# bghira/universal-metal-flash-attention

Measured on AMD Instinct MI355X. Metric: SDPA fwd TFLOPS (bf16) + int8 speedup, B=1 H=24 S=4096 D=128, 1/2/4/8 GPU, higher is better.
Workload: dtype bf16

## Files before the change

universal-metal-flash-attention_amd/csrc/fa_aux.hip:

```cpp
#include "fa_common.h"
#include "kernels.h"

namespace umfa {

template <typename T>
__global__ __launch_bounds__(256) void rope_rotate_kernel(RopeParams p) {
    const uint32_t chunks_per_row = p.D / 8;
    const uint64_t total = (uint64_t)p.B * p.H * p.S * chunks_per_row;
    for (uint64_t i = (uint64_t)blockIdx.x * 256 + threadIdx.x; i < total; i += (uint64_t)gridDim.x * 256) {
        const uint32_t ch = (uint32_t)(i % chunks_per_row);
        const uint64_t row = i / chunks_per_row;
        const uint32_t s = (uint32_t)(row % p.S);
        const uint64_t bh = row / p.S;
        const uint32_t h = (uint32_t)(bh % p.H), b = (uint32_t)(bh / p.H);
        const T* src = (const T*)p.src + (int64_t)b * p.src_batch_stride + (int64_t)h * p.src_head_stride +
                       (int64_t)s * p.src_seq_stride + ch * 8;
        T* dst = (T*)p.dst + row * p.D + ch * 8;
        const int64_t t = (int64_t)b * p.table_batch_stride + (int64_t)s * p.D + ch * 8;
        float x[8];
        if constexpr (sizeof(T) == 2) {
            typedef T T8 __attribute__((ext_vector_type(8)));
            const T8 v = *(const T8*)src;
#pragma unroll
            for (int j = 0; j < 8; ++j) x[j] = (float)v[j];
        } else {
            const f32x4 a = *(const f32x4*)src, c = *(const f32x4*)(src + 4);
#pragma unroll
            for (int j = 0; j < 4; ++j) { x[j] = a[j]; x[4 + j] = c[j]; }
        }
        const f32x4 c0 = *(const f32x4*)(p.cos_table + t), c1 = *(const f32x4*)(p.cos_table + t + 4);
        const f32x4 s0 = *(const f32x4*)(p.sin_table + t), s1 = *(const f32x4*)(p.sin_table + t + 4);
        float y[8];
        rope_rotate8(x, c0, c1, s0, s1, p.negate_sin != 0, y);
        if constexpr (sizeof(T) == 2) {
            typedef T T8 __attribute__((ext_vector_type(8)));
            T8 o;
#pragma unroll
            for (int j = 0; j < 8; ++j) o[j] = (T)y[j];
            *(T8*)dst = o;
        } else {
            *(f32x4*)dst = f32x4{y[0], y[1], y[2], y[3]};
            *(f32x4*)(dst + 4) = f32x4{y[4], y[5], y[6], y[7]};
        }
    }
}

template <typename T>
__global__ __launch_bounds__(256) void rope_rotate_pair_kernel(RopeParams p) {
    const uint32_t pairs = p.D / 2;
    const uint64_t total = (uint64_t)p.B * p.H * p.S * pairs;
    for (uint64_t i = (uint64_t)blockIdx.x * 256 + threadIdx.x; i < total; i += (uint64_t)gridDim.x * 256) {
        const uint32_t pr = (uint32_t)(i % pairs);
        const uint64_t row = i / pairs;
        const uint32_t s = (uint32_t)(row % p.S);
        const uint64_t bh = row / p.S;
        const uint32_t h = (uint32_t)(bh % p.H), b = (uint32_t)(bh / p.H);
        const T* src = (const T*)p.src + (int64_t)b * p.src_batch_stride + (int64_t)h * p.src_head_stride +
                       (int64_t)s * p.src_seq_stride + pr * 2;
        T* dst = (T*)p.dst + row * p.D + pr * 2;
        const int64_t t = (int64_t)b * p.table_batch_stride + (int64_t)s * p.D + pr * 2;
        const float c = p.cos_table[t];
        float sn = p.sin_table[t];
        if (p.negate_sin) sn = -sn;
        const float x0 = (float)src[0], x1 = (float)src[1];
        dst[0] = (T)(x0 * c - x1 * sn);
        dst[1] = (T)(x1 * c + x0 * sn);
    }
}

template <typename T>
static hipError_t launch_rope_t(const RopeParams& p, hipStream_t stream) {
    const bool vec = p.D % 8 == 0 && p.src_batch_stride % 8 == 0 && p.src_head_stride % 8 == 0 &&
                     p.src_seq_stride % 8 == 0 && p.table_batch_stride % 4 == 0 && ((uintptr_t)p.src & 15) == 0 &&
                     ((uintptr_t)p.dst & 15) == 0 && ((uintptr_t)p.cos_table & 15) == 0 && ((uintptr_t)p.sin_table & 15) == 0;
    const uint64_t work = (uint64_t)p.B * p.H * p.S * (vec ? p.D / 8 : p.D / 2);
    if (work == 0) return hipSuccess;
    const unsigned grid = (unsigned)((work + 255) / 256 < 2048 * 8 ? (work + 255) / 256 : 2048 * 8);
    if (vec) hipLaunchKernelGGL(rope_rotate_kernel<T>, dim3(grid), dim3(256), 0, stream, p);
    else hipLaunchKernelGGL(rope_rotate_pair_kernel<T>, dim3(grid), dim3(256), 0, stream, p);
    return hipGetLastError();
}

// ... 322 lines not shown
    if (wid >= total) return;
    const uint32_t tile = (uint32_t)(wid % T);
    const uint32_t rb = (uint32_t)((wid / T) % nrb64);
    const uint32_t slab = (uint32_t)(wid / ((uint64_t)T * nrb64));
    const uint32_t hm = slab % Hm, bm = slab / Hm;
    const uint8_t* base = (const uint8_t*)p.mask + (int64_t)bm * p.ms[0] + (int64_t)hm * p.ms[1];
    bool all_open = (uint64_t)tile * 64 + 64 <= p.Skv, any_open = false;
    uint32_t w[2];
    if constexpr (VEC16) {
        uint8_t* st = stage[wv];
        typedef unsigned u32x4 __attribute__((ext_vector_type(4)));
#pragma unroll
        for (int ps = 0; ps < 4; ++ps) {
            const uint32_t r = 16 * ps + (lane >> 2), c = lane & 3, row = rb * 64 + r, key0 = tile * 64 + 16 * c;
            u32x4 v = {0u, 0u, 0u, 0u};
            if (row < p.Sq && key0 < p.Skv) v = *(const u32x4*)(base + (int64_t)row * p.ms[2] + key0);
            *(u32x4*)(st + r * 80 + 16 * c) = v;
        }
        __builtin_amdgcn_fence(__ATOMIC_RELEASE, "wavefront");
        __builtin_amdgcn_wave_barrier();
        __builtin_amdgcn_fence(__ATOMIC_ACQUIRE, "wavefront");
#pragma unroll
        for (int qb = 0; qb < 2; ++qb) {
            const uint32_t r = 32 * qb + ql;
            uint32_t word = 0;
#pragma unroll
            for (int kb = 0; kb < 2; ++kb)
#pragma unroll
                for (int g = 0; g < 4; ++g) {
                    const uint32_t four = *(const uint32_t*)(st + r * 80 + 32 * kb + 8 * g + 4 * hi);
#pragma unroll
                    for (int e = 0; e < 4; ++e) word |= ((four >> (8 * e)) & 0xffu) ? 1u << (16 * kb + 4 * g + e) : 0u;
                }
            if (p.causal) word &= causal_word(rb * 64 + r, tile, hi);
            if (rb * 64 + r < p.Sq) {
                all_open = all_open && word == 0xffffffffu;
                any_open = any_open || word != 0;
            }
            w[qb] = word;
        }
    } else {
        const bool vec4 = p.ms[3] == 1 && ((p.ms[0] | p.ms[1] | p.ms[2]) & 3) == 0 && ((uintptr_t)p.mask & 3) == 0;
#pragma unroll
        for (int qb = 0; qb < 2; ++qb) {
            const uint32_t row = rb * 64 + 32 * qb + ql;
            uint32_t word = 0;
            if (row < p.Sq) {
                const uint8_t* rp = base + (int64_t)row * p.ms[2];
#pragma unroll
                for (int kb = 0; kb < 2; ++kb)
#pragma unroll
                    for (int g = 0; g < 4; ++g) {
                        const uint32_t key0 = tile * 64 + 32 * kb + 8 * g + 4 * hi;
                        uint32_t four = 0;
                        if (vec4 && key0 + 4 <= p.Skv) {
                            four = *(const uint32_t*)(rp + key0);
                        } else {
#pragma unroll
                            for (int e = 0; e < 4; ++e)
                                if (key0 + e < p.Skv) four |= (uint32_t)rp[(int64_t)(key0 + e) * p.ms[3]] << (8 * e);
                        }
#pragma unroll
                        for (int e = 0; e < 4; ++e) word |= ((four >> (8 * e)) & 0xffu) ? 1u << (16 * kb + 4 * g + e) : 0u;
                    }
                if (p.causal) word &= causal_word(row, tile, hi);
                all_open = all_open && word == 0xffffffffu;
                any_open = any_open || word != 0;
            }
            w[qb] = word;
        }
    }
    uint32_t* dst = bits + ((wid * 2) * 64 + lane);
    dst[0] = w[0];
    dst[64] = w[1];
    const bool open = __builtin_amdgcn_ballot_w64(any_open) != 0, full = __builtin_amdgcn_ballot_w64(!all_open) == 0;
    if (lane == 0) wflag[wid] = !open ? 1 : (full ? 2 : 0);
}

template <bool VEC16>
__global__ __launch_bounds__(256) void mask_pack_kernel(MaskPackArgs p) {
    mask_pack_body<VEC16>(p, blockIdx.x);
}

constexpr uint32_t VH_WORDS = 128, VH_DEPART = 64, VH_SCALE = 65, VH_AMAX = 66;
__device__ __forceinline__ int vscale_exponent(unsigned amax_bits) {
    if (amax_bits == 0) return 0;
    int E = (int)(amax_bits >> 7);
    E = E > 254 ? 254 : E;
    const int e = (E ? E - 127 : -126) - 15;
    return e < -100 ? -100 : e;
}
__device__ __forceinline__ unsigned bf16x8_amax(const unsigned (&r)[4], unsigned amax) {
#pragma unroll
    for (int j = 0; j < 4; ++j) {
        const unsigned a = r[j] & 0x7fff7fffu, m2 = (a & 0xffffu) > (a >> 16) ? (a & 0xffffu) : (a >> 16);
        amax = amax > m2 ? amax : m2;
    }
    return amax;
}
__device__ __forceinline__ unsigned wave_umax(unsigned x) {
#pragma unroll
    for (int off = 32; off > 0; off >>= 1) {
        const unsigned o2 = (unsigned)__shfl_xor((int)x, off, 64);
        x = x > o2 ? x : o2;
    }
    return x;
}
__device__ __forceinline__ unsigned block_amax(unsigned amax, unsigned* wmax) {
    amax = wave_umax(amax);
    if ((threadIdx.x & 63) == 0) wmax[threadIdx.x >> 6] = amax;
    __syncthreads();
    unsigned m = wmax[0];
    for (int w = 1; w < 4; ++w) m = m > wmax[w] ? m : wmax[w];
    return m;
}

struct CastRowsArgs {
    const uint16_t* src;
    int64_t sb, sh, ss;
    _Float16* dst;
    uint32_t H, S, D8, chunks;
    uint32_t* hdr;
    uint32_t wait_ticks;
};
template <int U, bool FUSED>
__device__ __forceinline__ void cast_rows_body(const CastRowsArgs& a, const uint32_t block) {
    const uint16_t* __restrict__ src = a.src;
    _Float16* __restrict__ dst = a.dst;
    uint32_t* __restrict__ hdr = a.hdr;
    const int64_t sb = a.sb, sh = a.sh, ss = a.ss;
    const uint32_t H = a.H, S = a.S, D8 = a.D8, chunks = a.chunks;
    typedef unsigned u32x4 __attribute__((ext_vector_type(4)));
    __shared__ unsigned wmax[4], slab_amax;
    const uint32_t bh = block / chunks, chunk = block - bh * chunks, b = bh / H, h = bh - b * H;
    const uint32_t rpw = 256u / D8;
    const uint32_t tr = threadIdx.x / D8, c = threadIdx.x - tr * D8;
    const uint32_t row0 = chunk * (U * rpw) + tr;
    const uint16_t* sp = src + (int64_t)b * sb + (int64_t)h * sh + 8 * c;
    _Float16* dp = dst + ((int64_t)bh * S) * (8 * D8) + 8 * c;
    uint32_t* const hw = hdr + VH_WORDS * (size_t)bh;
    u32x4 raw[U];
#pragma unroll
    for (int u = 0; u < U; ++u) {
        const uint32_t r = row0 + u * rpw;
        raw[u] = r < S && tr < rpw ? __builtin_nontemporal_load((const u32x4*)(sp + (int64_t)r * ss)) : u32x4{0, 0, 0, 0};
    }
    unsigned amax;
    if constexpr (FUSED) {
        amax = 0;
#pragma unroll
        for (int u = 0; u < U; ++u) {
            const unsigned r4[4] = {raw[u][0], raw[u][1], raw[u][2], raw[u][3]};
            amax = bf16x8_amax(r4, amax);
        }
        amax = block_amax(amax, wmax);
        if (threadIdx.x < 64) {
            if (threadIdx.x == 0) __hip_atomic_store(hw + chunk, 0x80000000u | amax, __ATOMIC_RELAXED, __HIP_MEMORY_SCOPE_AGENT);
            const uint64_t t_in = __builtin_amdgcn_s_memrealtime();
            unsigned f;
            bool served = true;
            for (;;) {
                f = threadIdx.x < chunks ? __hip_atomic_load(hw + threadIdx.x, __ATOMIC_RELAXED, __HIP_MEMORY_SCOPE_AGENT) : 0x80000000u;
                if (__builtin_amdgcn_ballot_w64((f & 0x80000000u) == 0) == 0) break;
                if (__builtin_amdgcn_s_memrealtime() - t_in >= a.wait_ticks) { served = false; break; }
                __builtin_amdgcn_s_sleep(2);
            }
            f = wave_umax(f & 0x7fffffffu);
            if (threadIdx.x == 0) slab_amax = served ? f : 0xffffffffu;
        }
        __syncthreads();
        if (slab_amax == 0xffffffffu) {
            for (uint32_t r = tr; r < S && tr < rpw; r += rpw) {
                const u32x4 v = *(const u32x4*)(sp + (int64_t)r * ss);
                const unsigned r4[4] = {v[0], v[1], v[2], v[3]};
                amax = bf16x8_amax(r4, amax);
            }
            __syncthreads();
            amax = block_amax(amax, wmax);
        } else {
            amax = slab_amax;
        }
    } else {
        amax = hw[VH_AMAX];
    }
    const int e = vscale_exponent(amax);
    const float mul = __uint_as_float((unsigned)(127 - e) << 23);
#pragma unroll
    for (int u = 0; u < U; ++u) {
        const uint32_t r = row0 + u * rpw;
        u32x4 o;
#pragma unroll
        for (int j = 0; j < 4; ++j) {
            const float lo = __uint_as_float(raw[u][j] << 16) * mul, hi = __uint_as_float(raw[u][j] & 0xffff0000u) * mul;
            asm("v_cvt_pk_f16_f32 %0, %1, %2" : "=v"(o[j]) : "v"(lo), "v"(hi));
        }
        if (r < S && tr < rpw) *(u32x4*)(dp + (int64_t)r * (8 * D8)) = o;
    }
    if (threadIdx.x < 64) {
        unsigned d = 0;
        if (threadIdx.x == 0) d = __hip_atomic_fetch_add(hw + VH_DEPART, 1u, __ATOMIC_RELAXED, __HIP_MEMORY_SCOPE_AGENT);
        d = (unsigned)__builtin_amdgcn_readfirstlane((int)d);
        if (d == chunks - 1) {
            if (FUSED && threadIdx.x < chunks) __hip_atomic_store(hw + threadIdx.x, 0u, __ATOMIC_RELAXED, __HIP_MEMORY_SCOPE_AGENT);
            if (threadIdx.x == 0) {
                hw[VH_SCALE] = (unsigned)(127 + e) << 23;
                __hip_atomic_store(hw + VH_DEPART, 0u, __ATOMIC_RELAXED, __HIP_MEMORY_SCOPE_AGENT);
                if (!FUSED) __hip_atomic_store(hw + VH_AMAX, 0u, __ATOMIC_RELAXED, __HIP_MEMORY_SCOPE_AGENT);
            }
        }
    }
}

template <int U, bool FUSED>
__global__ __launch_bounds__(256) void cast_rows_bf16_f16_kernel(CastRowsArgs a) {
    cast_rows_body<U, FUSED>(a, blockIdx.x);
}

template <int U, bool VEC16>
__global__ __launch_bounds__(256) void cast_rows_and_mask_pack_kernel(CastRowsArgs a, uint32_t cast_blocks, MaskPackArgs mk) {
    if (blockIdx.x < cast_blocks) cast_rows_body<U, true>(a, blockIdx.x);
    else mask_pack_body<VEC16>(mk, blockIdx.x - cast_blocks);
}

template <int U>
__global__ __launch_bounds__(256) void vamax_rows_kernel(const uint16_t* __restrict__ src, int64_t sb, int64_t sh, int64_t ss, uint32_t H, uint32_t S,
                                                         uint32_t D8, uint32_t chunks, uint32_t* __restrict__ hdr) {
    typedef unsigned u32x4 __attribute__((ext_vector_type(4)));
    __shared__ unsigned wmax[4];
    const uint32_t bh = blockIdx.x / chunks, chunk = blockIdx.x - bh * chunks, b = bh / H, h = bh - b * H;
    const uint32_t rpw = 256u / D8, tr = threadIdx.x / D8, c = threadIdx.x - tr * D8;
    const uint32_t row0 = chunk * (U * rpw) + tr;
    const uint16_t* sp = src + (int64_t)b * sb + (int64_t)h * sh + 8 * c;
    unsigned amax = 0;
#pragma unroll
    for (int u = 0; u < U; ++u) {
        const uint32_t r = row0 + u * rpw;
        const u32x4 v = r < S && tr < rpw ? *(const u32x4*)(sp + (int64_t)r * ss) : u32x4{0, 0, 0, 0};
        const unsigned r4[4] = {v[0], v[1], v[2], v[3]};
        amax = bf16x8_amax(r4, amax);
    }
    amax = block_amax(amax, wmax);
    if (threadIdx.x == 0 && amax) (void)__hip_atomic_fetch_max(hdr + VH_WORDS * (size_t)bh + VH_AMAX, amax, __ATOMIC_RELAXED, __HIP_MEMORY_SCOPE_AGENT);
}

template <int U>
static hipError_t launch_cast_rows_u(const void* src, const int64_t* strides, void* dst, uint32_t B, uint32_t H, uint32_t S, uint32_t D, uint32_t* hdr,
                                     hipStream_t stream, MaskPackArgs* mk) {
    const uint32_t D8 = D / 8, rpw = 256u / D8;
    const uint64_t chunks = ((uint64_t)S + U * rpw - 1) / (U * rpw), grid = (uint64_t)B * H * chunks;
    if (grid > 0x7fffffffull) return hipErrorInvalidValue;
    const bool fused = chunks <= 64 && !tuning().cast_two_pass.load(std::memory_order_relaxed);
    const CastRowsArgs a = {(const uint16_t*)src, strides[0], strides[1], strides[2], (_Float16*)dst, H, S, D8, (uint32_t)chunks, hdr,
                            (uint32_t)std::min<int64_t>(std::max(tuning().cast_wait_us.load(std::memory_order_relaxed), 0), 1000000) * 100u};
    if (fused) {
        if (mk && mk->total) {
            const unsigned g2 = (unsigned)((mk->total + 3) / 4);
            if (grid + g2 > 0x7fffffffull) return hipErrorInvalidValue;
            if (mk->vec16) hipLaunchKernelGGL((cast_rows_and_mask_pack_kernel<U, true>), dim3((unsigned)grid + g2), dim3(256), 0, stream, a, (unsigned)grid, *mk);
            else hipLaunchKernelGGL((cast_rows_and_mask_pack_kernel<U, false>), dim3((unsigned)grid + g2), dim3(256), 0, stream, a, (unsigned)grid, *mk);
            mk->done = true;
        } else {
            hipLaunchKernelGGL((cast_rows_bf16_f16_kernel<U, true>), dim3((unsigned)grid), dim3(256), 0, stream, a);
        }
    } else {
        hipLaunchKernelGGL(vamax_rows_kernel<U>, dim3((unsigned)grid), dim3(256), 0, stream, (const uint16_t*)src, strides[0], strides[1], strides[2], H, S,
                           D8, (uint32_t)chunks, hdr);
        hipLaunchKernelGGL((cast_rows_bf16_f16_kernel<U, false>), dim3((unsigned)grid), dim3(256), 0, stream, a);
    }
    return hipGetLastError();
}

static hipError_t launch_cast_rows_any(const void* src, const int64_t* strides, void* dst, uint32_t B, uint32_t H, uint32_t S, uint32_t D,
                                       uint32_t* hdr, hipStream_t stream, MaskPackArgs* mk) {
    if (!src || !dst || !hdr || (D & 7) || D > 2048 || strides[3] != 1 || (strides[0] | strides[1] | strides[2]) % 8 || ((uintptr_t)src & 15)) return hipErrorInvalidValue;
    if ((int64_t)B * H * S * D == 0) return hipSuccess;
    const uint32_t rpw = 256u / (D / 8);
    const uint64_t wg16 = (uint64_t)B * H * (((uint64_t)S + 16 * rpw - 1) / (16 * rpw));
    const int lab = tuning().cast_u.load(std::memory_order_relaxed);
    const uint64_t chunks16 = ((uint64_t)S + 16 * rpw - 1) / (16 * rpw);
    if (lab == 32 || (!lab && chunks16 > 64 && chunks16 <= 128)) return launch_cast_rows_u<32>(src, strides, dst, B, H, S, D, hdr, stream, mk);
    if (lab == 4 || (!lab && wg16 < (uint64_t)device_cu_count())) return launch_cast_rows_u<4>(src, strides, dst, B, H, S, D, hdr, stream, mk);
    return launch_cast_rows_u<16>(src, strides, dst, B, H, S, D, hdr, stream, mk);
}

hipError_t launch_bwd16_rowc(const float* lse, const float* dvec, float* rowc, int64_t n, const float* d_mul, hipStream_t stream) {
    if (n == 0) return hipSuccess;
    const unsigned grid = (unsigned)((n + 255) / 256 < 4096 ? (n + 255) / 256 : 4096);
    hipLaunchKernelGGL(bwd16_rowc_kernel, dim3(grid), dim3(256), 0, stream, lse, dvec, rowc, n, d_mul);
    return hipGetLastError();
}

hipError_t launch_dequant(const DequantParams& p, hipStream_t stream) {
    if (!p.src || (!p.dst && !p.dst16) || p.H_src == 0 || p.H_dst % p.H_src) return hipErrorInvalidValue;
    const int64_t n = (int64_t)p.B * p.H_dst * p.S * p.D;
// ... 612 lines not shown
```

universal-metal-flash-attention_amd/csrc/fa_common.h:

```cpp
#pragma once
#include <hip/hip_runtime.h>
#include <stdint.h>

namespace umfa {

typedef float f32x16 __attribute__((ext_vector_type(16)));
typedef float f32x4 __attribute__((ext_vector_type(4)));
typedef short s16x8 __attribute__((ext_vector_type(8)));
typedef short s16x4 __attribute__((ext_vector_type(4)));
typedef _Float16 f16x8 __attribute__((ext_vector_type(8)));
typedef __bf16 bf16x8 __attribute__((ext_vector_type(8)));
typedef int i32x4 __attribute__((ext_vector_type(4)));
typedef int i32x16 __attribute__((ext_vector_type(16)));

enum Prec : int { P_FP16 = 0, P_BF16 = 1, P_FP32 = 2, P_INT8 = 3, P_INT4 = 4 };
enum MaskKind : int { MK_NONE = 0, MK_BOOL = 1, MK_F32 = 2, MK_F16 = 3, MK_BF16 = 4,
                      MK_WINDOW = 5  };

#define UMFA_LOG2E 1.4426950408889634f
#define UMFA_LN2 0.6931471805599453f

struct FwdParams {
    const void* q;
    const void* k;
    const void* v;
    void* o;
    float* lse;
    const void* mask;
    int64_t qs[4], ks[4], vs[4];
    int64_t os[2];
    int64_t ms[4];
    uint32_t B, H, Sq, Skv, D;
    float scale;
    int causal;
    int mask_kind;
    int in_prec;
    int out_prec;
    uint32_t n_full;
    uint32_t nsplit;
    float* part_buf;
    uint32_t* part_cnt;
    const uint8_t* mask_flags;
    uint32_t mf_bs, mf_hs;
    uint32_t mf_nrb, mf_ntiles;
    uint32_t win_left, win_right;
    const uint32_t* mk_bits;
    const uint32_t* mk_list;
    const uint32_t* mk_cnt;
    uint32_t mk_bs, mk_hs, mk_nrb64, mk_T;
    const uint32_t* mk_prefix;
    const float* rope_cos;
    const float* rope_sin;
    int64_t rope_tb;
    int pv16;
    const float* vsc;
    uint32_t vsc_bs, vsc_hs;
    uint32_t decode_form;
    uint32_t cbal;
    uint32_t cbal_delta;
    const uint32_t* guard;
    uint32_t guard_want;
    uint32_t mask_padded;
};

__device__ __forceinline__ void rope_rotate8(const float (&x)[8], const f32x4& c0, const f32x4& c1, const f32x4& s0,
                                             const f32x4& s1, bool negate_sin, float (&y)[8]) {
    const float cs[4] = {c0[0], c0[2], c1[0], c1[2]};
    float sn[4] = {s0[0], s0[2], s1[0], s1[2]};
#pragma unroll
    for (int k = 0; k < 4; ++k) {
        if (negate_sin) sn[k] = -sn[k];
        y[2 * k] = __builtin_fmaf(x[2 * k], cs[k], -__fmul_rn(x[2 * k + 1], sn[k]));
        y[2 * k + 1] = __builtin_fmaf(x[2 * k + 1], cs[k], __fmul_rn(x[2 * k], sn[k]));
    }
#pragma unroll
    for (int j = 0; j < 8; ++j) asm volatile("" : "+v"(y[j]));
}

template <typename T, typename V8>
__device__ __forceinline__ V8 rope_fragment(V8 v, const float* __restrict__ cos_t, const float* __restrict__ sin_t, int64_t at) {
    float x[8], y[8];
#pragma unroll
    for (int j = 0; j < 8; ++j) x[j] = (float)v[j];
    const f32x4 c0 = *(const f32x4*)(cos_t + at), c1 = *(const f32x4*)(cos_t + at + 4);
    const f32x4 s0 = *(const f32x4*)(sin_t + at), s1 = *(const f32x4*)(sin_t + at + 4);
    rope_rotate8(x, c0, c1, s0, s1, false, y);
    V8 o;
#pragma unroll
    for (int j = 0; j < 8; ++j) o[j] = (T)y[j];
    return o;
}

struct BwdParams {
    const void* dout;
    const void* q;
    const void* k;
    const void* v;
    const float* o;
    const float* lse;
    float* dq;
    float* dk;
    float* dv;
    float* dvec;
    float* rowc;
    const void* mask;
    uint32_t B, H, Sq, Skv, D;
    float scale;
    int causal;
    int in_prec;
    int dout_prec;
    int grad_in_type;
    int o_in_type;
    int phases;
    uint32_t Hkv;
    int dkdv_fp32;
    void* ds;
    int ds_lab;
    const float* units;
    int64_t ms[4];
    int mask_kind;
    uint32_t win_left, win_right;
    const uint8_t* mask_flags;
    uint32_t mf_bs, mf_hs, mf_nrb, mf_ntiles;
};

inline void bwd_dense_f32_mask(BwdParams& p, const void* mask) {
    p.mask = mask;
    p.mask_kind = mask ? MK_F32 : MK_NONE;
    p.ms[3] = 1;
    p.ms[2] = p.Skv;
    p.ms[1] = (int64_t)p.Sq * p.Skv;
    p.ms[0] = (int64_t)p.H * p.Sq * p.Skv;
}

__device__ __forceinline__ float unit_c(const BwdParams& p) { return p.units ? p.units[0] : 1.0f; }
__device__ __forceinline__ float unit_dq(const BwdParams& p) { return p.units ? p.units[1] : 1.0f; }
__device__ __forceinline__ float unit_dk(const BwdParams& p) { return p.units ? p.units[2] : 1.0f; }
__device__ __forceinline__ float unit_dv(const BwdParams& p) { return p.units ? p.units[3] : 1.0f; }
__device__ __forceinline__ float unit_rowd(const BwdParams& p) { return p.units ? p.units[4] : 1.0f; }
__device__ __forceinline__ float unit_dvec(const BwdParams& p) { return p.units ? p.units[5] : 1.0f; }
__device__ __forceinline__ int unit_exponent(unsigned amax_bits) {
    if (amax_bits == 0 || amax_bits >= 0x7f800000u) return 0;
    const int E = (int)(amax_bits >> 23);
    const int e = (E ? E : 1) - 127;
    return e < -126 ? -126 : e > 126 ? 126 : e;
// ... 48 lines not shown
```

universal-metal-flash-attention_amd/csrc/fa_fwd16_w64.hip:

```cpp
#include <algorithm>
#include <cmath>
#include <cstdlib>
#include <type_traits>

#include "fa_fwd16_w64_params.h"

namespace umfa {

#define W64_I8 0
#define W64_BODY_INC "fa_fwd16_w64_body.inc"
#define W64_T __bf16
#define W64_MFMA "v_mfma_f32_32x32x16_bf16"
#define W64_MFMA_QK "v_mfma_f32_32x32x16_bf16"
#define W64_MSUM "v_mfma_f32_4x4x4_16b_bf16"
#define W64_ONES_BITS 0x3f803f80u
#define W64_LAZY_PARTS 1
#define W64_CVT "v_cvt_pk_bf16_f32"
#define W64_KERNEL fa_fwd16_w64_bf16
#include "fa_fwd16_w64_kernel.inc"
#undef W64_T
#undef W64_MFMA
#undef W64_MFMA_QK
#undef W64_MSUM
#undef W64_ONES_BITS
// ... 261 lines not shown
        if (p.out_prec != P_FP32 && p.out_prec != p.in_prec) return false;
        if (p.ms[3] != 1) return false;
        if (!mask_needs_copy(p)) {
            if (((uintptr_t)p.mask & 15) != 0 || (p.ms[0] & 7) != 0 || (p.ms[1] & 7) != 0 || (p.ms[2] & 7) != 0) return false;
        } else if (tuning().no_w64_ragged_mask.load(std::memory_order_relaxed) && p.mask_kind == MK_F16) {
            return false;
        }
        if (p.mask_kind != MK_F32 && p.ms[2] != 0 && (uint64_t)p.ms[2] * 2 * 64 > 0x7fffffffull) return false;
        if (mask_copy_bytes(p) > ((size_t)1 << 30)) return false;
        if (p.mask_kind == MK_F32) {
            if (tuning().no_w64_f32_mask.load(std::memory_order_relaxed)) return false;
            const int ratio = tuning().f32_mask_ratio.load(std::memory_order_relaxed);
            if (ratio > 0) {
                const uint64_t Bm = p.ms[0] != 0 ? p.B : 1, Hm = p.ms[1] != 0 ? p.H : 1, eb = 2;
                const uint64_t mask_bytes = Bm * Hm * p.Sq * p.Skv * 4, qkvo = (uint64_t)p.B * p.H * p.D * ((uint64_t)p.Sq * (eb + 4) + 2ull * p.Skv * eb);
                if (mask_bytes > (uint64_t)ratio * qkvo) return false;
            } else if (!mask_flags_worthwhile(p)) {
                return false;
            }
        }
        if (w64_grid(p) > 512u) return false;
        if (tuning().force_w64.load(std::memory_order_relaxed)) return true;
        const uint64_t blocks = (uint64_t)p.B * p.H * ((p.Sq + 255) / 256), cus = (uint64_t)w64_cu_count();
        return blocks >= cus;
    }
    if (p.mask_kind == MK_BOOL) {
        if (tuning().no_w64_mask.load(std::memory_order_relaxed) || !p.mask || (p.D != 128 && p.D != 64) || p.rope_cos) return false;
        if (p.in_prec == P_BF16 && !p.pv16) return false;
        if (p.Skv < 64 || p.Sq < 256 || (p.Sq % 256 != 0 && p.Sq < 1024) || ((p.Skv + 63) / 64) > 1024u) return false;
        if (p.out_prec != P_FP32 && p.out_prec != p.in_prec) return false;
        const uint64_t blocks = (uint64_t)p.B * p.H * ((p.Sq + 255) / 256), cus = (uint64_t)w64_cu_count();
        if (w64_grid(p) > 512u) return false;
        if (tuning().force_w64.load(std::memory_order_relaxed)) return true;
        if (p.causal) return false;
        if (p.in_prec == P_BF16 && p.Sq < 1024) return false;
        if (p.in_prec == P_BF16 && p.Sq < 2048 && ((p.ms[0] == 0 && p.ms[1] == 0) || p.ms[2] == 0)) return false;
        return blocks >= cus || (p.ms[2] == 0 && blocks * ((p.Skv + 63) / 64) >= cus * 10) || ((p.ms[0] != 0 || p.ms[1] != 0) && blocks * 8 >= cus * 3);
    }
    if (w64_is_window(p) && p.rope_cos) return false;
    if (p.D == 64 && p.rope_cos) return false;
    if (p.Skv < 64 || p.Sq < 256 || (p.Sq % 256 != 0 && p.Sq < 1024)) return false;
    if (p.out_prec != P_FP32 && p.out_prec != p.in_prec) return false;
    if (!tuning().force_w64.load(std::memory_order_relaxed)) {
        if (w64_is_window(p)) {
            const uint64_t cus = (uint64_t)w64_cu_count(), nqb = (p.Sq + 255) / 256;
            const uint64_t items = (uint64_t)p.B * p.H * nqb, steps = items * w64_tiles_per_item(p);
            if (items % cus != 0 && steps < cus * 10) return false;
        } else if (!(fwd_w64_predict_us(p) < fwd_16_predict_us(p))) {
            return false;
        }
    }
    return true;
}

static uint32_t w64_grid(const FwdParams& p) {
    if (p.mask_kind == MK_BOOL || p.mask_kind == MK_F16 || p.mask_kind == MK_BF16) {
        const uint64_t items = (uint64_t)p.B * p.H * ((p.Sq + 255) / 256);
        const uint64_t cus = (uint64_t)w64_cu_count();
        if (const int gi = tuning().w64_grid.load(std::memory_order_relaxed)) {
            if (gi > 0 && (uint64_t)gi <= cus && (uint64_t)gi <= items && gi <= 512) return (uint32_t)gi;
        }
        const uint64_t gmax = cus < 512 ? cus : 512;
        if (items < cus) return (uint32_t)((p.ms[2] == 0 && items * ((p.Skv + 63) / 64) >= cus * 10) ? gmax : items);
        return (uint32_t)gmax;
    }
    const bool pairs = p.causal && !w64_is_window(p);
    uint64_t total = (uint64_t)p.B * p.H * ((p.Sq + 255) / 256) * w64_tiles_per_item(p);
    if (pairs) total = (uint64_t)p.B * p.H * (((p.Sq + 255) / 256 + 1) / 2);
    const uint32_t cus = (uint32_t)w64_cu_count();
    if (const int gi = tuning().w64_grid.load(std::memory_order_relaxed)) {
        const uint32_t g = (uint32_t)gi;
        if (gi > 0 && g <= cus && g <= total) return g;
    }
    if (!pairs) {
        const uint64_t items = (uint64_t)p.B * p.H * ((p.Sq + 255) / 256);
        if (items < cus && cus / items >= 2 && items * (cus / items) <= total) return (uint32_t)(items * (cus / items));
        if (items < cus && 2 * (uint64_t)w64_tiles_per_item(p) * (cus - items) < 35 * cus) return (uint32_t)items;
    }
    return total < cus ? (uint32_t)total : cus;
}

uint32_t fwd_w64_grid(const FwdParams& p) { return w64_grid(p); }

FwdW64Plan fwd_w64_plan(const FwdParams& p) {
    FwdW64Plan plan;
    const uint32_t items = p.B * p.H * ((p.Sq + 255) / 256);
    (void)items;
    plan.cnt_bytes = ((size_t)w64_grid(p) * sizeof(uint32_t) + 255) & ~(size_t)255;
    plan.buf_bytes = (size_t)2 * w64_grid(p) * (4 * 2 * 17 * 1024);
    return plan;
}

template <typename KFN>
static hipError_t launch_w64_kernel(KFN kfn, const FwdParams& p, const W64Params& wp, hipStream_t stream) {
    const uint32_t grid = w64_grid(p);
    const size_t lds = 65536 + 4 * 32 * (512 + 16) + 64 + 4096 + 8192 + 2048 + 64;
    if (hipError_t e = ensure_dynamic_lds((const void*)kfn, lds); e != hipSuccess) return e;
    hipLaunchKernelGGL(kfn, dim3(grid), dim3(256), lds, stream, wp);
    return hipGetLastError();
}

hipError_t launch_fwd_w64(const FwdParams& p, float* part_buf, uint32_t* part_cnt, hipStream_t stream, const char** name) {
    if (!fwd_w64_supported(p) || !part_buf || !part_cnt) return hipErrorNotSupported;
    W64Params wp;
    wp.q = p.q; wp.k = p.k; wp.v = p.v; wp.o = p.o; wp.lse = p.lse;
    for (int i = 0; i < 3; ++i) { wp.qs[i] = p.qs[i]; wp.ks[i] = p.ks[i]; wp.vs[i] = p.vs[i]; }
    wp.B = p.B; wp.H = p.H; wp.Sq = p.Sq; wp.Skv = p.Skv;
    wp.scale = p.scale;
    wp.n_items = p.B * p.H * ((p.Sq + 255) / 256);
    wp.T = (p.Skv + 63) / 64;
    wp.part_buf = part_buf;
    wp.part_cnt = part_cnt;
    w64_softmax_policy(p.in_prec, &wp.tau, &wp.lazy);
    wp.skew = (uint32_t)tuning().w64_skew.load(std::memory_order_relaxed);
    if (tuning().w64_skew.load(std::memory_order_relaxed) == -1) wp.skew = 0xffffffffu;
    wp.rope_cos = p.rope_cos; wp.rope_sin = p.rope_sin; wp.rope_tb = p.rope_tb;
    wp.vsc = p.vsc; wp.vsc_bs = p.vsc_bs; wp.vsc_hs = p.vsc_hs;
    if (p.in_prec == P_BF16 && p.pv16 && !p.vsc) return hipErrorInvalidValue;
    wp.Tw = wp.T; wp.win_left = wp.win_right = 0;
    const bool rope = p.rope_cos != nullptr, window = w64_is_window(p), fp32o = p.out_prec == P_FP32, maska = p.mask_kind == MK_F16, maskt = p.mask_kind == MK_BOOL || maska;
    wp.mask = nullptr; wp.mask_s[0] = wp.mask_s[1] = wp.mask_s[2] = 0;
    wp.guard = maska ? p.guard : nullptr;
    if (p.guard && (!maska || p.guard_want != 0u)) return hipErrorInvalidValue;
    if (maskt) {
        if ((!maska && !p.mk_bits) || !p.mk_list || !p.mk_cnt) return hipErrorInvalidValue;
        if (maska) { wp.mask = p.mask; wp.mask_s[0] = p.ms[0]; wp.mask_s[1] = p.ms[1]; wp.mask_s[2] = p.ms[2]; }
        wp.mk_bits = p.mk_bits; wp.mk_list = p.mk_list; wp.mk_cnt = p.mk_cnt;
        wp.mk_bs = p.mk_bs; wp.mk_hs = p.mk_hs; wp.mk_nrb64 = p.mk_nrb64;
        wp.mk_prefix = p.mk_prefix;
#ifndef W64_LAB_MASK_FORCE_LAZY
        if (p.ms[2] != 0 || p.causal || tuning().no_w64_mask_lazy.load(std::memory_order_relaxed)) wp.lazy = 0;
#endif
    }
    if (rope && p.out_prec != p.in_prec) return hipErrorNotSupported;
    if (window) {
        wp.Tw = w64_tiles_per_item(p);
        wp.win_left = (int32_t)w64_win_left(p);
        wp.win_right = (int32_t)w64_win_right(p);
    }
#define W64_FAMILY(FAM, T16, HAS_ROPE)                                                                                         \
    do {                                                                                                                       \
        if constexpr (HAS_ROPE >= 2) {        \
            if (maskt) return fp32o ? launch_w64_kernel(FAM<float, false, false, false, true>, p, wp, stream) : launch_w64_kernel(FAM<T16, false, false, false, true>, p, wp, stream); \
        }                                                                                                                      \
        if constexpr (HAS_ROPE == 1 || HAS_ROPE == 2) {                                                                        \
            if (rope) return p.causal ? launch_w64_kernel(FAM<T16, true, true>, p, wp, stream) : launch_w64_kernel(FAM<T16, false, true>, p, wp, stream); \
        }                                                                                                                      \
        if (window) return fp32o ? launch_w64_kernel(FAM<float, false, false, true>, p, wp, stream) : launch_w64_kernel(FAM<T16, false, false, true>, p, wp, stream); \
        if (p.causal) return fp32o ? launch_w64_kernel(FAM<float, true>, p, wp, stream) : launch_w64_kernel(FAM<T16, true>, p, wp, stream); \
        return fp32o ? launch_w64_kernel(FAM<float, false>, p, wp, stream) : launch_w64_kernel(FAM<T16, false>, p, wp, stream); \
    } while (0)
    static const char* const names[3][2][3] = {
        {{"fa_fwd16_w64<bf16,128>", "fa_fwd16_w64<bf16,128,rope>", "fa_fwd16_w64<bf16,128,window>"},
         {"fa_fwd16_w64<bf16,64>", "fa_fwd16_w64<bf16,64,rope>", "fa_fwd16_w64<bf16,64,window>"}},
        {{"fa_fwd16_w64<bf16,128,pv16>", "fa_fwd16_w64<bf16,128,pv16,rope>", "fa_fwd16_w64<bf16,128,pv16,window>"},
         {"fa_fwd16_w64<bf16,64,pv16>", "fa_fwd16_w64<bf16,64,pv16,rope>", "fa_fwd16_w64<bf16,64,pv16,window>"}},
        {{"fa_fwd16_w64<fp16,128>", "fa_fwd16_w64<fp16,128,rope>", "fa_fwd16_w64<fp16,128,window>"},
         {"fa_fwd16_w64<fp16,64>", "fa_fwd16_w64<fp16,64,rope>", "fa_fwd16_w64<fp16,64,window>"}}};
    if (p.D == 64 && rope) return hipErrorNotSupported;
    const int fam = p.in_prec == P_BF16 ? (p.pv16 ? 1 : 0) : 2;
    if (maskt && fam == 0) return hipErrorNotSupported;
    if (maska && fam == 0) return hipErrorNotSupported;
    if (maska) {
        *name = p.D == 64 ? (fam == 1 ? "fa_fwd16_w64<bf16,64,pv16,bias>" : "fa_fwd16_w64<fp16,64,bias>") : (fam == 1 ? "fa_fwd16_w64<bf16,128,pv16,bias>" : "fa_fwd16_w64<fp16,128,bias>");
        return launch_fwd_w64_bias(wp, fam, fp32o, w64_grid(p), 65536 + 4 * 32 * (512 + 16) + 64 + 4096 + 8192 + 2048 + 64, stream, (int)p.D);
    }
    *name = maska ? (fam == 1 ? "fa_fwd16_w64<bf16,128,pv16,bias>" : "fa_fwd16_w64<fp16,128,bias>") : maskt ? (p.D == 64 ? (fam == 1 ? "fa_fwd16_w64<bf16,64,pv16,mask>" : "fa_fwd16_w64<fp16,64,mask>")
                               : (fam == 1 ? "fa_fwd16_w64<bf16,128,pv16,mask>" : "fa_fwd16_w64<fp16,128,mask>"))
                  : names[fam][p.D == 64 ? 1 : 0][rope ? 1 : window ? 2 : 0];
    if (p.D == 64) {
        if (fam == 0) W64_FAMILY(fa_fwd16_w64d64_bf16, __bf16, 0);
        if (fam == 1) W64_FAMILY(fa_fwd16_w64d64_bf16pv16, __bf16, 3);
        W64_FAMILY(fa_fwd16_w64d64_f16, _Float16, 3);
    }
    if (fam == 0) W64_FAMILY(fa_fwd16_w64_bf16, __bf16, 1);
    if (fam == 1) W64_FAMILY(fa_fwd16_w64_bf16pv16, __bf16, 2);
    W64_FAMILY(fa_fwd16_w64_f16, _Float16, 2);
#undef W64_FAMILY
}

bool fwd_w64_i8_supported(const FwdParams& p) {
    if (tuning().no_w64.load(std::memory_order_relaxed) || p.D != 128) return false;
    if (!(p.scale > 0.0f)) return false;
    if (p.Skv < 64 || p.Sq < 256 || (p.Sq % 256 != 0 && p.Sq < 1024)) return false;
    if (p.mask_kind == MK_BOOL && p.mask) {
        if (tuning().no_w64_mask.load(std::memory_order_relaxed) || p.causal) return false;
        if (((p.Skv + 63) / 64) > 1024u || w64_grid(p) > 512u) return false;
        if (tuning().force_w64.load(std::memory_order_relaxed)) return true;
        const uint64_t blocks = (uint64_t)p.B * p.H * ((p.Sq + 255) / 256), cus = (uint64_t)w64_cu_count();
        return blocks >= cus || (p.ms[2] == 0 && blocks * ((p.Skv + 63) / 64) >= cus * 10) || ((p.ms[0] != 0 || p.ms[1] != 0) && blocks * 8 >= cus * 3);
    }
    return p.mask_kind == MK_NONE && !p.mask;
}

hipError_t launch_fwd_w64_i8(const FwdParams& p, const QuantViews& v, float* part_buf, uint32_t* part_cnt, hipStream_t stream) {
    if (!fwd_w64_i8_supported(p) || !part_buf || !part_cnt || v.dpq != 128) return hipErrorNotSupported;
    W64I8Params wp;
    wp.q8 = v.q8; wp.k8 = v.k8; wp.v16 = (const _Float16*)v.v16;
    wp.v8 = v.v8; wp.v_e8 = v.v_e8;
    wp.q_scale = v.q_scale; wp.k_scale = v.k_scale;
    wp.o = p.o; wp.lse = p.lse;
// ... 29 lines not shown
```

universal-metal-flash-attention_amd/csrc/fa_fwd16_w64_kernel.inc:

```

#ifdef W64_ABL_NOBAR
#define W64_ITER_BARRIER() asm volatile("" ::: "memory")
#elif defined(W64_LAB_WAITSTAMP)
#define W64_ITER_BARRIER()                                                                         \
    do {                                                                                           \
        asm volatile("s_waitcnt lgkmcnt(0)" ::: "memory");                                         \
        const unsigned long long w0_ = __builtin_amdgcn_s_memtime();                               \
        asm volatile("s_waitcnt vmcnt(0) lgkmcnt(0)" ::: "memory");                                \
        const unsigned long long w1_ = __builtin_amdgcn_s_memtime();                               \
        asm volatile("s_waitcnt lgkmcnt(0)\n\ts_barrier" ::: "memory");                            \
        const unsigned long long w2_ = __builtin_amdgcn_s_memtime();                               \
        asm volatile("s_waitcnt lgkmcnt(0)" ::: "memory");                                         \
        st_wait += w1_ - w0_;                                                                      \
        st_bar += w2_ - w1_;                                                                       \
    } while (0)
#elif defined(W64_ABL_VMCNT8)
#define W64_ITER_BARRIER() asm volatile("s_waitcnt vmcnt(8) lgkmcnt(0)\n\ts_barrier" ::: "memory")
#else
#define W64_ITER_BARRIER() asm volatile("s_waitcnt vmcnt(0) lgkmcnt(0)\n\ts_barrier" ::: "memory")
#endif
#ifdef W64_ABL_NODMA
#define W64_DMA_ON 0
#else
#define W64_DMA_ON 1
#endif
#ifdef W64_FORCE_MASKED
#define W64_MASKED_TILE(i) true
#else
#define W64_MASKED_TILE(i) (MASKT ? mk_class(i) != 2u : ((CAUSAL && tile_at(i) >= diag0) || (WINDOW && win_edge(tile_at(i))) || (ktail && tile_at(i) == T_ - 1)))
#endif
#ifdef W64_ABL_NONMSEL
#define W64_NMSEL 0
#else
#define W64_NMSEL 1
#endif
#ifdef W64_MIDBAR
#define W64_END_BARRIER(KNEXT) do { } while (0)
#else
#ifdef W64_LAB_NOKF
#define W64_END_BARRIER(KNEXT) W64_ITER_BARRIER()
#else
#define W64_END_BARRIER(KNEXT)                                                            \
    do {                                                                                  \
        W64_ITER_BARRIER();                                                               \
        _Pragma("unroll") for (int ks = 0; ks < 4; ++ks) kf[0][ks] = k_frag(KNEXT, ks);   \
    } while (0)
#endif
#endif
#ifndef W64_SPEC
#define W64_SPEC 1
#endif
#ifdef W64_NO_RESCALE
#define W64_RESCALE_ON 0
#else
#define W64_RESCALE_ON 1
#endif

#ifndef W64_F8
#define W64_F8 0
#endif
#ifndef W64_DP
#define W64_DP 128
#endif
#ifndef W64_MSUM_ON
#define W64_MSUM_ON 0
#endif
#if W64_I8 && !defined(W64_I8_NOBIAS)
#define W64_NVGPR (W64_F8 ? 96 : 112)
#else
#define W64_NVGPR (W64_MSUM_ON ? 118 : 128)
#endif
#if W64_I8
template <typename OUT, bool CAUSAL, bool MASKT = false>
__global__ __launch_bounds__(256, 1) __attribute__((amdgpu_num_vgpr(W64_NVGPR))) void W64_KERNEL(W64I8Params p) {
    static_assert(!(MASKT && (CAUSAL || W64_F8)), "mask-tensor instantiation of the int8 kernel: plain sweep over the block's tile list, fp16 P V");
    constexpr bool WINDOW = false;
    constexpr bool MASKA = false;
    (void)MASKA;
    typedef i32x4 KF;
    constexpr int KS = 4;
    constexpr int KSLOT = 8192;
#else
template <typename OUT, bool CAUSAL, bool ROPE = false, bool WINDOW = false, bool MASKT = false, bool MASKA = false>
__global__ __launch_bounds__(256, 1) __attribute__((amdgpu_num_vgpr(W64_NVGPR))) void W64_KERNEL(W64Params p) {
    static_assert(!(WINDOW && (CAUSAL || ROPE)), "window instantiations: no causal pairing, no fused rotation");
    static_assert(!(MASKT && (CAUSAL || ROPE || WINDOW)), "mask-tensor instantiations: plain sweep over the block's tile list");
#ifndef W64_MADD
#define W64_MADD 0
#endif
    static_assert(!MASKA || (MASKT && W64_MADD), "additive mask tensors: a mask-tensor instantiation of a bias family (head_dim 128 or 64)");
    static_assert(MASKA || !W64_MADD, "the bias families exist for their MASKA instantiations only");
    constexpr int KS = W64_DP / 16;
    constexpr int KSLOT = 64 * 2 * W64_DP;
    static_assert(W64_DP == 128 || (W64_DP == 64 && !ROPE), "head_dim 128, or 64 without the fused rotation");
#endif
    typedef W64_T T;
    typedef Mma16<T> M;
    typedef typename M::V8 V8;
    typedef typename M::V4 V4;
#if !W64_I8
    typedef V8 KF;
#endif
    typedef unsigned u32x4_t __attribute__((ext_vector_type(4)));
    constexpr int NDB = W64_DP / 32;
    constexpr int ROW_IN = 2 * W64_DP;
    constexpr int VSLOT = W64_F8 ? 8192 : 64 * ROW_IN;
    constexpr int VRING = W64_I8 ? 32768 : 2 * KSLOT;
    const float TAU = p.tau;
#if !W64_I8
    if constexpr (MASKA) {
        if (p.guard != nullptr && *p.guard != 0u) return;
    }
#endif

    extern __shared__ __attribute__((aligned(16))) char smem[];
    const int tid = threadIdx.x, lane = tid & 63, ql = lane & 31, hi = lane >> 5;
    const int uw = __builtin_amdgcn_readfirstlane(tid >> 6);
    const uint32_t lds0 = (uint32_t)(size_t)((LDS_AS char*)smem);
#ifndef W64_LAZY_PARTS
#define W64_LAZY_PARTS 0
#endif
#if W64_MSUM_ON && !W64_F8
    ms_init_ones(W64_ONES_BITS);
#define W64_L_ZERO() ms_zero_l()
#define W64_L_SCALE(A0, A1) ms_scale_l((A0), (A1))
#define W64_L_READ(L0, L1) ms_read_l((L0), (L1))
#elif !W64_F8
#define W64_L_ZERO() do { _Pragma("unroll") for (int j_ = 0; j_ < 4; ++j_) l4[0][j_] = l4[1][j_] = 0.0f; } while (0)
#define W64_L_SCALE(A0, A1) do { _Pragma("unroll") for (int j_ = 0; j_ < 4; ++j_) { l4[0][j_] *= (A0); l4[1][j_] *= (A1); } } while (0)
#define W64_L_READ(L0, L1) ((L0) = (l4[0][0] + l4[0][1]) + (l4[0][2] + l4[0][3]), (L1) = (l4[1][0] + l4[1][1]) + (l4[1][2] + l4[1][3]))
#endif
#if W64_LAZY_PARTS
    const bool lazy_on = p.lazy != 0;
    bool force_exact = false;
#ifndef W64_LAZY_HI16
#define W64_LAZY_HI16 0x1p10f
#endif
    constexpr float LAZY_HI = W64_LAZY_PARTS == 2 ? W64_LAZY_HI16 : 0x1p30f, LAZY_OVF = W64_LAZY_PARTS == 2 ? 0x1p15f : 0x1p100f;
    constexpr float LAZY_LOST = W64_LAZY_PARTS == 2 ? 0x1p-6f : 0x1p-100f;
    constexpr unsigned OVF_FLAG_OFF = 65536u + 4u * 32u * (512u + 16u);
    if (threadIdx.x == 0) *(volatile uint32_t LDS_AS*)(uintptr_t)(lds0 + OVF_FLAG_OFF) = 0u;
    __builtin_amdgcn_s_waitcnt(0xc07f);
#endif

    auto tr_read_at = [](unsigned addr) -> V4 {
// ... 171 lines not shown
        _Pragma("unroll") for (int k_ = 1; k_ < (n); ++k_) fs_acc[k_] += (uint32_t)fs_now[k_] - (uint32_t)fs_now[k_ - 1]; \
        fs_last = (uint32_t)fs_now[(n) - 1];                                                        \
        fs_valid = true;                                                                            \
        ++fs_tiles;                                                                                 \
    } while (0)
#endif
#ifdef W64_LAB_STAMPS
    const unsigned long long st_rt0 = __builtin_amdgcn_s_memrealtime(), st_ck0 = __builtin_amdgcn_s_memtime();
    unsigned long long st_pro = 0, st_loop = 0, st_drain = 0, st_epi = 0, st_t = 0, st_wait = 0, st_bar = 0;
#define W64_STAMP(acc) do { const unsigned long long now_ = __builtin_amdgcn_s_memtime(); acc += now_ - st_t; st_t = now_; } while (0)
#else
#define W64_STAMP(acc) do { } while (0)
#endif

    uint32_t ntail = 0;
    bool tail_first = false;
    if (s_end > s_begin) {
        const uint32_t it0 = item_of_step(s_begin), it1 = item_of_step(s_end - 1);
        ntail = it1 - it0 + 1;
        tail_first = item_start(it0) != s_begin;
    }
    const uint32_t my_jobs = CAUSAL ? (n_jobs > w ? (n_jobs - w + G - 1) / G : 0u) : 0u;
    const uint32_t nseg = CAUSAL ? 2 * my_jobs : full_rounds + ntail;

    auto make_srd = [&](const void* base, uint32_t bytes) {
        const unsigned long long a = (unsigned long long)base;
        i32x4 d;
        d[0] = __builtin_amdgcn_readfirstlane((int)(a & 0xffffffffu));
        d[1] = __builtin_amdgcn_readfirstlane((int)((a >> 32) & 0xffffu));
        d[2] = __builtin_amdgcn_readfirstlane((int)bytes);
        d[3] = 0x00020000;
        return d;
    };
    auto seg_decode = [&](uint32_t si_, uint32_t& item_, uint32_t& t0_, uint32_t& n_, uint32_t& litem_, bool& desc_) -> bool {
        litem_ = 0;
        desc_ = false;
        if constexpr (CAUSAL) {
            const uint32_t job = (si_ >> 1) * G + w, jbh = job / jobs_per_head, jj = job % jobs_per_head;
            desc_ = (si_ & 1) != 0;
            const uint32_t q = desc_ ? nqb - 1 - jj : jj;
            if (desc_ && q == jj) return false;
            item_ = jbh * nqb + q;
            t0_ = 0;
            n_ = item_tiles(item_);
        } else {
            const bool is_tail = tail_first ? (si_ < ntail) : (si_ >= full_rounds);
            if (is_tail) {
                const uint32_t ti = tail_first ? si_ : si_ - full_rounds;
                litem_ = item_of_step(s_begin) + ti;
                const uint64_t ist = item_start(litem_), ien = MASKT ? item_start(litem_ + 1) : ist + Tst;
                const uint64_t sb = ist > s_begin ? ist : s_begin, se = ien < s_end ? ien : s_end;
                t0_ = (uint32_t)(sb - ist);
                n_ = (uint32_t)(se - sb);
                item_ = full_rounds * G + litem_;
            } else {
                item_ = (tail_first ? si_ - ntail : si_) * G + w;
                if (item_ >= p.n_items) return false;
                t0_ = 0;
                n_ = MASKT ? item_tiles(item_) : Tst;
            }
        }
        return true;
    };
#ifndef W64_MFMA16
#define W64_MFMA16 "v_mfma_f32_16x16x32_bf16"
#endif
#ifndef W64_PREFETCH_NEXT
#define W64_PREFETCH_NEXT 0
#endif
#if W64_PREFETCH_NEXT
    static_assert(!WINDOW, "the prefetch computes the next segment's first tile without the window offset");
    KF qf[2][KS];
    int kdma[4];
    bool have_pref = false;
#endif
#if W64_I8
    constexpr bool ROPE_ON = false;
    (void)ROPE_ON;
#else
    constexpr bool ROPE_ON = ROPE;
    (void)ROPE_ON;
#endif

    for (uint32_t si = 0; si < nseg; ++si) {
        int tid_s = tid;
        if constexpr (MASKA) asm volatile("" : "+v"(tid_s));
        const int lane = tid_s & 63, ql = lane & 31, hi = lane >> 5;
#ifdef W64_LAB_STAMPS
        if (si) { asm volatile("s_waitcnt vmcnt(0)" ::: "memory"); W64_STAMP(st_epi); }
#endif
        uint32_t item, t0, n, litem = 0;
        bool desc = false;
#if W64_LAZY_PARTS
        bool lazy = lazy_on && !force_exact;
        force_exact = false;
        bool ovf = false;
#endif
        if (!seg_decode(si, item, t0, n, litem, desc)) continue;
#if !W64_PREFETCH_NEXT
        KF qf[2][KS];
        int kdma[4];
        constexpr bool have_pref = false;
#endif
        auto issue_q_k0 = [&](uint32_t item_, uint32_t tfirst_, int k_step_) {
            const uint32_t bh_ = item_ / nqb, qblk_ = item_ % nqb;
            const uint32_t q0_ = qblk_ * 256 + (uint32_t)uw * 64;
#if W64_I8
            const int8_t* qp_ = p.q8 + (int64_t)bh_ * p.Sq * 128;
            const int8_t* kp_ = p.k8 + (int64_t)bh_ * p.Skv * 128;
            const auto q_rsrc_ = __builtin_amdgcn_make_buffer_rsrc((void*)qp_, 0, (int)(p.Sq * 128u), 0x00020000);
            const i32x4 k_srd_ = make_srd(kp_, p.Skv * 128u);
#else
            const uint32_t b_ = bh_ / p.H, h_ = bh_ % p.H;
            const T* qp_ = (const T*)p.q + ((int64_t)b_ * p.qs[0] + (int64_t)h_ * p.qs[1]);
            const T* kp_ = (const T*)p.k + ((int64_t)b_ * p.ks[0] + (int64_t)h_ * p.ks[1]);
            const auto q_rsrc_ = __builtin_amdgcn_make_buffer_rsrc((void*)qp_, 0, (int)((p.Sq - 1) * (uint32_t)q_stride_b + ROW_IN), 0x00020000);
            const i32x4 k_srd_ = make_srd(kp_, (p.Skv - 1) * (uint32_t)k_stride_b + ROW_IN);
#endif
#pragma unroll
            for (int j = 0; j < 4; ++j) kdma[j] = kdma0[j] + (int)tfirst_ * k_step0;
#pragma unroll
            for (int j = 0; j < (W64_I8 ? 2 : W64_DP / 32); ++j) {
                asm volatile("s_mov_b32 m0, %0\n\ts_nop 0\n\tbuffer_load_dwordx4 %1, %2, 0 offen lds"
                             ::"s"(lds_wave_k + j * 1024), "v"(kdma[j]), "s"(k_srd_) : "memory");
                kdma[j] += k_step_;
            }
#pragma unroll
            for (int qb = 0; qb < 2; ++qb) {
                const int qoff = (int)(q0_ + 32 * qb + ql) * q_stride_b + 16 * hi;
#pragma unroll
                for (int ks = 0; ks < KS; ++ks)
                    qf[qb][ks] = __builtin_bit_cast(KF, __builtin_amdgcn_raw_buffer_load_b128(q_rsrc_, qoff + 32 * ks, 0, 0));
            }
        };
        const uint32_t Ti = item_tiles(item);
        const uint32_t bh = item / nqb, qblk = item % nqb;
        const uint32_t b = bh / p.H, h = bh % p.H;
        const uint32_t q0 = qblk * 256 + (uint32_t)uw * 64;

#if W64_I8
        (void)b; (void)h;
        const int8_t* qp = p.q8 + (int64_t)bh * p.Sq * 128;
        const int8_t* kp = p.k8 + (int64_t)bh * p.Skv * 128;
#if W64_F8
        const uint8_t* vp = p.v8 + (int64_t)bh * T_ * 8192;
        const uint32_t* __restrict__ vexp = p.v_e8 + (int64_t)bh * p.nkblk;
        const i32x4 v_srd = make_srd(vp, T_ * 8192u);
#else
        const _Float16* vp = p.v16 + (int64_t)bh * p.Skv * 128;
        const i32x4 v_srd = make_srd(vp, p.Skv * 256u);
#endif
        const auto q_rsrc = __builtin_amdgcn_make_buffer_rsrc((void*)qp, 0, (int)(p.Sq * 128u), 0x00020000);
        const i32x4 k_srd = make_srd(kp, p.Skv * 128u);
        const float sq = (q0 < p.Sq ? p.q_scale[(int64_t)bh * p.nqblk + q0 / 64] : 0.0f) * p.scale * UMFA_LOG2E;
        const float* __restrict__ ksc = p.k_scale + (int64_t)bh * p.nkblk;
        int sc_win = -1;
        float ksc_w = 0.0f;
#if W64_F8
        unsigned vexp_w = 0x7f7f7f7fu;
#endif
        auto load_scale_window = [&](uint32_t tile) {
            const int win = (int)(tile >> 6);
            if (win != sc_win) {
                sc_win = win;
                const uint32_t t = ((uint32_t)win << 6) + (uint32_t)lane;
                ksc_w = t < p.nkblk ? ksc[t] : 0.0f;
#if W64_F8
                vexp_w = t < p.nkblk ? vexp[t] : 0x7f7f7f7fu;
#endif
                __builtin_amdgcn_s_waitcnt(0x0F70);
            }
        };
        auto k_scale_of = [&](uint32_t tile) -> float {
            load_scale_window(tile);
            return __builtin_bit_cast(float, __builtin_amdgcn_readlane(__builtin_bit_cast(int, ksc_w), (int)(tile & 63u)));
        };
#ifndef W64_I8_NOBIAS
        float kmax = 0.0f;
        for (uint32_t t = lane; t < p.nkblk; t += 64) kmax = fmaxf(kmax, ksc[t]);
#pragma unroll
        for (int off = 32; off > 0; off >>= 1) kmax = fmaxf(kmax, __shfl_xor(kmax, off, 64));
        const float bias_bound = fmaxf(I8_BIAS * 1.25f * sq * kmax, 0x1p-60f);
        const int eb = ((__builtin_bit_cast(int, bias_bound) >> 23) & 0xff) - 126;
        const float mgrid = __builtin_bit_cast(float, (eb - 24 + 127) << 23), inv_mgrid = __builtin_bit_cast(float, (24 - eb + 127) << 23);
        const float cgrid = __builtin_bit_cast(float, (eb - 46 + 127) << 23), inv_cgrid = __builtin_bit_cast(float, (46 - eb + 127) << 23);
#define W64_C2(x) (__builtin_rintf((x) * inv_cgrid) * cgrid)
#define W64_MGRID(x) (__builtin_ceilf((x) * inv_mgrid) * mgrid)
#if W64_LAZY_PARTS
        lazy = lazy && eb <= 24;
#endif
#else
#define W64_C2(x) (x)
#define W64_MGRID(x) (x)
#endif
#else
#define W64_MGRID(x) (x)
        const T* qp = (const T*)p.q + ((int64_t)b * p.qs[0] + (int64_t)h * p.qs[1]);
        const T* kp = (const T*)p.k + ((int64_t)b * p.ks[0] + (int64_t)h * p.ks[1]);
        const T* vp = (const T*)p.v + ((int64_t)b * p.vs[0] + (int64_t)h * p.vs[1]);
        const auto q_rsrc = __builtin_amdgcn_make_buffer_rsrc((void*)qp, 0, (int)((p.Sq - 1) * (uint32_t)q_stride_b + ROW_IN), 0x00020000);
        const i32x4 k_srd = make_srd(kp, (p.Skv - 1) * (uint32_t)k_stride_b + ROW_IN);
        const i32x4 v_srd = make_srd(vp, (p.Skv - 1) * (uint32_t)v_stride_b + ROW_IN);
#endif

        uint32_t toff = 0;
        if constexpr (WINDOW) {
            const uint32_t blk0 = qblk * 256u;
            const uint32_t lo = blk0 > (uint32_t)win_left ? (blk0 - (uint32_t)win_left) / 64u : 0u;
            toff = lo < T_ - Tst ? lo : T_ - Tst;
        }
        uint32_t tfirst = toff + (desc ? n - 1 : t0);
        int k_step = desc ? -k_step0 : k_step0, v_step = desc ? -v_step0 : v_step0;
        const int dm_step = desc ? -64 : 64;
        const uint32_t* __restrict__ mk_lst = MASKT ? p.mk_list + (uint64_t)(mk_slab(bh) * nqb + qblk) * T_ * 2 : nullptr;
        constexpr unsigned MK_LIST_OFF = 65536u + 4u * 32u * (512u + 16u) + 64u + 4096u;
        const unsigned mk_list_lds = lds0 + MK_LIST_OFF;
        uint32_t mk_tile = 0, mk_cls = 2, mk_next = 0;
        uint32_t mk_ncls = 0;
        (void)mk_ncls;
        auto mk_class = [&](uint32_t) -> uint32_t { return mk_cls; };
        auto tile_at = [&](uint32_t i) -> uint32_t {
// ... 83 lines not shown
                asm volatile("s_mov_b32 m0, %0\n\ts_nop 0\n\tbuffer_load_dword %1, %2, 0 offen lds\n\t"
                             "buffer_load_dword %1, %2, 0 offen offset:256 lds"
                             :: "s"(dst), "v"(voff), "s"(mk_srd) : "memory");
            }
        };
        auto mk_take = [&](uint32_t i) {
            if constexpr (MASKT && !MASKA) {
                const unsigned a = mk_ring + (i & 1u) * 512u + (unsigned)lane * 4u;
                mwc[0] = *(const unsigned LDS_AS*)(uintptr_t)a;
                mwc[1] = *(const unsigned LDS_AS*)(uintptr_t)(a + 256u);
            }
        };
        (void)mtmp;
        if constexpr (MASKT) {
            asm volatile("s_barrier" ::: "memory");
            for (uint32_t j = (uint32_t)tid; j < 2 * n; j += 256u) *(unsigned LDS_AS*)(uintptr_t)(mk_list_lds + 4u * j) = mk_lst[2 * t0 + j];
            __builtin_amdgcn_s_waitcnt(0x0F70);
            asm volatile("s_waitcnt lgkmcnt(0)\n\ts_barrier" ::: "memory");
            mk_steps(0);
            tfirst = mk_tile;
            k_step = ((int)mk_next - (int)mk_tile) * k_step0;
        }
        auto win_edge = [&](uint32_t t) -> bool {
            const int64_t k0_ = 64 * (int64_t)t;
            return k0_ + 63 > (int64_t)q0 + win_right || k0_ + win_left < (int64_t)q0 + 63;
        };
        (void)win_edge;
        int vdma[4];
#pragma unroll
        for (int j = 0; j < 4; ++j) vdma[j] = vdma0[j] + (int)tfirst * v_step0;

#ifdef W64_LAB_STAMPS
        st_t = __builtin_amdgcn_s_memtime();
#endif
        asm volatile("s_barrier" ::: "memory");
        mk_request(0, tfirst);
        KF kf[2][KS];
#if !W64_I8
        if constexpr (ROPE) {
#pragma unroll
            for (int j = 0; j < 4; ++j) kdma[j] = kdma0[j] + (int)tfirst * k_step0;
#pragma unroll
            for (int j = 0; j < 4; ++j) {
                asm volatile("s_mov_b32 m0, %0\n\ts_nop 0\n\tbuffer_load_dwordx4 %1, %2, 0 offen lds"
                             ::"s"(lds_wave_k + j * 1024), "v"(kdma[j]), "s"(k_srd) : "memory");
                kdma[j] += k_step;
            }
            const unsigned qst = lds0 + 65536u + (unsigned)uw * (32 * (512 + 16));
#pragma unroll 4
            for (int it = 0; it < 16; ++it) {
                const int r = it * 4 + (lane >> 4), c = lane & 15;
                const uint32_t row = q0 + (uint32_t)r;
                const V8 v = __builtin_bit_cast(V8, __builtin_amdgcn_raw_buffer_load_b128(q_rsrc, (int)row * q_stride_b + 16 * c, 0, 0));
                const int64_t at = (int64_t)b * p.rope_tb + (int64_t)(row < p.Sq ? row : 0) * 128 + 8 * c;
                const V8 o = rope_fragment<T, V8>(v, p.rope_cos, p.rope_sin, at);
                *(V8 LDS_AS*)(uintptr_t)(qst + (unsigned)(r * 256 + ((c ^ (r & 15)) << 4))) = o;
            }
            __builtin_amdgcn_fence(__ATOMIC_RELEASE, "wavefront");
            __builtin_amdgcn_wave_barrier();
            __builtin_amdgcn_fence(__ATOMIC_ACQUIRE, "wavefront");
#pragma unroll
            for (int qb = 0; qb < 2; ++qb) {
                const int r = 32 * qb + ql;
#pragma unroll
                for (int ks = 0; ks < KS; ++ks)
                    qf[qb][ks] = *(const V8 LDS_AS*)(uintptr_t)(qst + (unsigned)(r * 256 + (((2 * ks + hi) ^ (r & 15)) << 4)));
            }
        } else
#endif
        {
            (void)q_rsrc;
            if (!have_pref) issue_q_k0(item, tfirst, k_step);
        }
#if W64_PREFETCH_NEXT
        have_pref = false;
#endif
        zero_o();
#if !W64_F8
#if !W64_MSUM_ON
        float l4[2][4];
#endif
        W64_L_ZERO();
#endif
        asm volatile("s_waitcnt vmcnt(0)\n\ts_barrier" ::: "memory");
        __builtin_amdgcn_s_waitcnt(0x0F70);
#pragma unroll
        for (int ks = 0; ks < 4; ++ks) kf[0][ks] = k_frag(0, ks);

#if W64_F8
        i32x8 vf8[4];
        f8_zero_l();
#else
        V8 vf[4][NDB];
#endif
        float mr[2] = {-INFINITY, -INFINITY}, mo[2] = {-INFINITY, -INFINITY}, nm[2] = {0.f, 0.f}, mx[2][2] = {{0.f, 0.f}, {0.f, 0.f}};
        bool pending = false;
        float em[2] = {0.f, 0.f};
        int dmask[2], dleft = 0;
        {
            constexpr int NEVER = -(1 << 28);
#ifdef W64_FORCE_MASKED
            const int causal_term = NEVER;
#else
            const int diag_term = (int)(64 * tfirst) + 4 * hi - (int)q0 - ql;
            const int causal_term = CAUSAL ? diag_term : WINDOW ? diag_term - win_right : NEVER;
            if constexpr (WINDOW) dleft = diag_term + win_left;
#endif
#pragma unroll
            for (int qb = 0; qb < 2; ++qb) {
                const int tail_term = ktail ? (int)(64 * tfirst) + 4 * hi - (int)p.Skv + 1 + 32 * qb : NEVER;
                dmask[qb] = causal_term > tail_term ? causal_term : tail_term;
            }
        }
        (void)dleft;
        const float neg_inf = -INFINITY;
        const uint32_t diag0 = 4 * qblk;

#if W64_I8 && !defined(W64_I8_NOBIAS)
#define W64_UNBIAS(x) ((x) - I8_BIAS)
#define W64_SET_NMB() (nmb[0] = __builtin_fmaf(-I8_BIAS, c2, nm[0]), nmb[1] = __builtin_fmaf(-I8_BIAS, c2, nm[1]))
#else
#define W64_UNBIAS(x) (x)
#define W64_SET_NMB() ((void)0)
#endif
#define W64_DECIDE()                                                                                            \
    do {                                                                                                        \
        const float mc0 = W64_UNBIAS(max_xor32(fmaxf(mx[0][0], mx[0][1]))) * c2;                                \
        const float mc1 = W64_UNBIAS(max_xor32(fmaxf(mx[1][0], mx[1][1]))) * c2;                                \
        pending = __builtin_amdgcn_ballot_w64((mc0 - mr[0] > TAU) | (mc1 - mr[1] > TAU)) != 0;                  \
        mo[0] = mr[0];                                                                                          \
        mo[1] = mr[1];                                                                                          \
        mr[0] = pending ? W64_MGRID(fmaxf(mr[0], mc0)) : mr[0];                                                 \
        mr[1] = pending ? W64_MGRID(fmaxf(mr[1], mc1)) : mr[1];                                                 \
         \
        nm[0] = (W64_NMSEL && SPARSE && mr[0] == -INFINITY) ? 0.0f : -mr[0];                                                 \
        nm[1] = (W64_NMSEL && SPARSE && mr[1] == -INFINITY) ? 0.0f : -mr[1];                                                 \
        W64_SET_NMB();                                                                                          \
    } while (0)

#if W64_F8
#define W64_SCALE_LACC(A0, A1) f8_scale_l((A0), (A1))
#define W64_SET_VSC(T) (load_scale_window(T), f8_set_vscale((unsigned)__builtin_amdgcn_readlane((int)vexp_w, (int)((T) & 63u))))
#else
#define W64_SCALE_LACC(A0, A1) W64_L_SCALE((A0), (A1))
#define W64_SET_VSC(T) ((void)0)
#endif
#define W64_DECIDE2()                                                                                           \
    do {                                                                                                        \
        em[0] = max_xor32(fmaxf(mx[0][0], mx[0][1]));                                                           \
        em[1] = max_xor32(fmaxf(mx[1][0], mx[1][1]));                                                           \
         \
        pending = __builtin_amdgcn_ballot_w64((em[0] > TAU) | (em[1] > TAU) |                                   \
                                              (SPARSE && ((mr[0] == -INFINITY && em[0] > -INFINITY) |           \
                                                          (mr[1] == -INFINITY && em[1] > -INFINITY)))) != 0;    \
    } while (0)
#define W64_MOVE_REF(FIX)                                                                                       \
    do {                                                                                                        \
        const float mc0 = em[0] - nm[0], mc1 = em[1] - nm[1];      \
        mo[0] = mr[0];                                                                                          \
        mo[1] = mr[1];                                                                                          \
        mr[0] = W64_MGRID(fmaxf(mr[0], mc0));                                                                   \
        mr[1] = W64_MGRID(fmaxf(mr[1], mc1));                                                                   \
        const float n0 = (W64_NMSEL && SPARSE && mr[0] == -INFINITY) ? 0.0f : -mr[0];                           \
        const float n1 = (W64_NMSEL && SPARSE && mr[1] == -INFINITY) ? 0.0f : -mr[1];                           \
        FIX(n0 - nm[0], n1 - nm[1]);                                                                            \
        nm[0] = n0;                                                                                             \
        nm[1] = n1;                                                                                             \
// ... 419 lines not shown
                };
                pub_db(std::integral_constant<int, 0>{});
                pub_db(std::integral_constant<int, 1>{});
                if constexpr (W64_I8 || W64_DP == 128) {
                    pub_db(std::integral_constant<int, 2>{});
                    pub_db(std::integral_constant<int, 3>{});
                }
                __builtin_amdgcn_raw_buffer_store_b128(__builtin_bit_cast(u32x4_t, f32x4{lt[qb] > 0.0f ? mr[qb] : -INFINITY, lt[qb], 0.0f, 0.0f}), prsrc,
                                                       (int)(mine + (qb * 17 + 16) * 1024), 0, 16);
            };
            publish_qb(std::integral_constant<int, 0>{});
            publish_qb(std::integral_constant<int, 1>{});
            asm volatile("s_waitcnt vmcnt(0)" ::: "memory");
            __syncthreads();
            if (tid == 0) flag_s[1] = __hip_atomic_fetch_add(p.part_cnt + litem, 1u, __ATOMIC_RELAXED, __HIP_MEMORY_SCOPE_AGENT);
            __syncthreads();
            folder = flag_s[1] == nparts - 1;
        }
        if (!folder) continue;
        if (tid == 0) __hip_atomic_store(p.part_cnt + litem, 0u, __ATOMIC_RELAXED, __HIP_MEMORY_SCOPE_AGENT);
        __builtin_amdgcn_fence(__ATOMIC_ACQUIRE, "wavefront");

        auto fold_qb = [&](auto QBC) {
            constexpr int qb = decltype(QBC)::value;
            const float m_own = lt[qb] > 0.0f ? mr[qb] : -INFINITY;
            float mm = m_own;
            for (uint32_t j = 0; j < nparts; ++j) {
                if (j == j_own) continue;
                const f32x4 ml = __builtin_bit_cast(f32x4, __builtin_amdgcn_raw_buffer_load_b128(prsrc, (int)(slot_off(j) + (qb * 17 + 16) * 1024), 0, 16));
                mm = fmaxf(mm, ml[0]);
            }
            float ll = 0.0f;
            const uint32_t q_row = q0 + 32 * qb + ql;
            auto fold_half = [&](auto HC) {
                constexpr int h2 = decltype(HC)::value;
                float acc[32];
#pragma unroll
                for (int r = 0; r < 32; ++r) acc[r] = 0.0f;
                float lsum = 0.0f;
                for (uint32_t j = 0; j < nparts; ++j) {
                    float x[32], mj, lj;
                    if (j == j_own) {
                        float t0[16], t1[16];
                        if constexpr (qb == 0) { read_o0<2 * h2>(t0); read_o0<2 * h2 + 1>(t1); } else { read_o1<2 * h2>(t0); read_o1<2 * h2 + 1>(t1); }
#pragma unroll
                        for (int r = 0; r < 16; ++r) { x[r] = t0[r]; x[16 + r] = t1[r]; }
                        mj = m_own;
                        lj = lt[qb];
                    } else {
                        const uint32_t so = slot_off(j) + qb * 17 * 1024;
                        f32x4 c[8];
#pragma unroll
                        for (int k = 0; k < 8; ++k)
                            c[k] = __builtin_bit_cast(f32x4, __builtin_amdgcn_raw_buffer_load_b128(prsrc, (int)(so + (8 * h2 + k) * 1024), 0, 16));
                        const f32x4 ml = __builtin_bit_cast(f32x4, __builtin_amdgcn_raw_buffer_load_b128(prsrc, (int)(so + 16 * 1024), 0, 16));
#pragma unroll
                        for (int k = 0; k < 8; ++k)
#pragma unroll
                            for (int e = 0; e < 4; ++e) x[4 * k + e] = c[k][e];
                        mj = ml[0];
                        lj = ml[1];
                    }
                    const float wj = (SPARSE && mj == -INFINITY) ? 0.0f : __builtin_amdgcn_exp2f(mj - mm);
                    lsum += wj * lj;
#pragma unroll
                    for (int r = 0; r < 32; ++r) acc[r] += wj * x[r];
                }
                ll = lsum;
                const float inv = ((WINDOW || MASKT) && !(lsum > 0.0f)) ? 0.0f : (1.0f / lsum) * vsc;
                float b0[16], b1[16];
#pragma unroll
                for (int r = 0; r < 16; ++r) { b0[r] = acc[r]; b1[r] = acc[16 + r]; }
                stage_block(2 * h2, b0, inv);
                stage_block(2 * h2 + 1, b1, inv);
            };
            fold_half(std::integral_constant<int, 0>{});
            if constexpr (W64_I8 || W64_DP == 128) fold_half(std::integral_constant<int, 1>{});
            flush_rows(qb);
            if (p.lse && hi == 0 && q_row < p.Sq) p.lse[(int64_t)bh * p.Sq + q_row] = (mm + log2f(ll)) * UMFA_LN2;
        };
        fold_qb(std::integral_constant<int, 0>{});
        fold_qb(std::integral_constant<int, 1>{});
    }
#ifdef W64_LAB_STAMPS
    asm volatile("s_waitcnt vmcnt(0)" ::: "memory");
    W64_STAMP(st_epi);
    asm volatile("s_barrier" ::: "memory");
    if (tid == 0 && p.lse) {
        unsigned long long* dbg = (unsigned long long*)p.lse + (size_t)blockIdx.x * 8;
        dbg[4] = st_pro;
        dbg[5] = st_loop;
#if defined(W64_LAB_FSTAMP)
        dbg[4] = ((unsigned long long)fs_acc[1] << 32) | fs_acc[0];
        dbg[5] = ((unsigned long long)fs_acc[3] << 32) | fs_acc[2];
        dbg[6] = ((unsigned long long)fs_acc[5] << 32) | fs_acc[4];
        dbg[7] = ((unsigned long long)fs_acc[7] << 32) | fs_acc[6];
        (void)st_wait; (void)st_bar; (void)fs_tiles;
#elif defined(W64_LAB_GAPSTAMP)
        dbg[4] = st_g[0]; dbg[5] = st_g[1];
        dbg[6] = st_g[2];
        dbg[7] = st_g[3];
        (void)st_wait; (void)st_bar;
#elif defined(W64_LAB_WAITSTAMP) || defined(W64_LAB_DMASTAMP)
        dbg[6] = st_wait;
        dbg[7] = st_bar;
#else
        (void)st_wait; (void)st_bar;
        dbg[6] = st_drain;
        dbg[7] = st_epi;
#endif
        dbg[0] = st_rt0;
        dbg[1] = __builtin_amdgcn_s_memrealtime();
        dbg[2] = st_ck0;
        dbg[3] = __builtin_amdgcn_s_memtime();
    }
#endif
}
#ifdef W64_L_ZERO
#undef W64_L_ZERO
#undef W64_L_SCALE
#undef W64_L_READ
#endif
#undef W64_NVGPR
```

universal-metal-flash-attention_amd/csrc/fa_fwd16_w64_params.h:

```cpp
#pragma once
#include <cstdint>

#include "fa_common.h"
#include "fa_fwd_16_kernel.h"
#include "kernels.h"

namespace umfa {

struct W64Params {
    const void* q;
    const void* k;
    const void* v;
    void* o;
    float* lse;
    int64_t qs[3], ks[3], vs[3];
    uint32_t B, H, Sq, Skv;
    float scale;
    uint32_t n_items, T;
    float* part_buf;
    uint32_t* part_cnt;
    float tau;
    uint32_t lazy;
    uint32_t skew;
    uint32_t Tw;
    int32_t win_left, win_right;
    const float* rope_cos;
    const float* rope_sin;
    int64_t rope_tb;
    const uint32_t* mk_bits;
    const uint32_t* mk_list;
    const uint32_t* mk_cnt;
    uint32_t mk_bs, mk_hs, mk_nrb64;
    const uint32_t* mk_prefix;
    const void* mask;
    int64_t mask_s[3];
    const float* vsc;
    uint32_t vsc_bs, vsc_hs;
    const uint32_t* guard;
};

#include "fa_fwd16_w64_regs.inc"

__device__ __forceinline__ constexpr int k8_off_128(int row, int ch) { return row * 128 + 16 * (ch ^ ((row >> 1) & 7)); }

struct W64I8Params {
    const int8_t* q8;
    const int8_t* k8;
    const _Float16* v16;
    const uint8_t* v8;
    const uint32_t* v_e8;
    const float* q_scale;
    const float* k_scale;
    void* o;
    float* lse;
    uint32_t B, H, Sq, Skv, nqblk, nkblk;
    float scale;
    uint32_t n_items, T;
    float* part_buf;
    uint32_t* part_cnt;
    float tau;
    uint32_t lazy;
    uint32_t skew;
    const uint32_t* mk_bits;
    const uint32_t* mk_list;
    const uint32_t* mk_cnt;
    uint32_t mk_bs, mk_hs, mk_nrb64;
    const float* vsc;
};

hipError_t launch_fwd_w64_bias(const W64Params& wp, int family, bool fp32_out, uint32_t grid, size_t lds, hipStream_t stream, int head_dim);

}
```

universal-metal-flash-attention_amd/csrc/kernels.h:

```cpp
#pragma once
#include <hip/hip_runtime.h>

#include <atomic>

#include "fa_common.h"

namespace umfa {

enum SoftmaxRef : int {
    SM_DEFAULT = 0,
    SM_EXACT = 1,
    SM_DEFERRED = 2,
    SM_LAZY = 3,
};
struct Tuning {
    std::atomic<int> sm_mode{SM_DEFAULT};
    std::atomic<float> sm_tau{6.0f};
    std::atomic<int> force_w64{0}, no_w64{0}, w64_grid{0}, w64_skew{0}, no_mask_flags{0}, bwd_exact{0}, bwd_dq{0}, bwd_persist{0},
        bwd_separate_delta{0}, no_split{0}, force_split{0}, no_dma{0}, bn64{0}, pv_fp16{0}, bwd_ds_store{0}, no_w64_mask{0}, ksplit{0}, no_pipe{0}, no_w64_mask_lazy{0}, no_w64_bias{0}, no_w64_f32_mask{0} ,
        no_mask_realign{0} ,
        no_w64_ragged_mask{0} ,
        mask_pass_ratio{0} ,
        f32_mask_ratio{0} ,
        cast_two_pass{0} , bwd_ds_lab{0} ,
        cast_u{0} ,
        quant_block_wg{0} ,
        cast_wait_us{100} ,
        decode_ks{0} ,
        cbal{0} ,
        cbal_delta{-1} ,
        sync_chunks{1} ,
        sync_chunked_calls{0} ,
        mirror_cache_hits{0} ,
        no_bwd_mask{0} ,
        sdpa_dropout{0} ;
};
Tuning& tuning();
bool set_tuning(const char* name, const char* value);
bool get_tuning(const char* name, char* out, size_t n);
int device_cu_count();
hipError_t ensure_dynamic_lds(const void* kernel, size_t bytes);

hipError_t launch_fwd_exact(const FwdParams& p, hipStream_t stream, const char** name);

hipError_t launch_fwd_wide(const FwdParams& p, hipStream_t stream, const char** name);
hipError_t launch_bwd_wide(const BwdParams& p, hipStream_t stream, const char** name);

hipError_t launch_fwd_16(const FwdParams& p, hipStream_t stream, const char** name);
bool fwd_16_supported(const FwdParams& p);
struct FwdSplitPlan {
    uint32_t n_full, nsplit;
    size_t buf_bytes, cnt_bytes;
    uint32_t decode = 0;
    uint32_t cbal = 0, cbal_delta = 0;
};
FwdSplitPlan fwd_16_split_plan(const FwdParams& p);

struct FwdW64Plan {
    size_t buf_bytes, cnt_bytes;
};
bool fwd_w64_supported(const FwdParams& p);
uint32_t fwd_w64_grid(const FwdParams& p);
double fwd_w64_predict_us(const FwdParams& p);
double fwd_16_predict_us(const FwdParams& p);
FwdW64Plan fwd_w64_plan(const FwdParams& p);
hipError_t launch_fwd_w64(const FwdParams& p, float* part_buf, uint32_t* part_cnt, hipStream_t stream, const char** name);

hipError_t launch_bwd(const BwdParams& p, hipStream_t stream, const char** name);
bool bwd_16_supported(const BwdParams& p);
hipError_t launch_bwd_16(const BwdParams& p, hipStream_t stream, const char** name);
bool bwd_16_mask_supported(const BwdParams& p);
hipError_t launch_bwd_16_masked(const BwdParams& p, hipStream_t stream, const char** name);

struct DropFwdParams : FwdParams {
    const int64_t* rng;
    uint32_t thresh;
    float dscale;
};
struct DropBwdParams : BwdParams {
    const int64_t* rng;
    uint32_t thresh;
    float dscale;
};
bool fwd_16_dropout_supported(const FwdParams& p);
hipError_t launch_fwd_16_dropout(const DropFwdParams& p, hipStream_t stream, const char** name);
bool bwd_16_dropout_supported(const BwdParams& p);
hipError_t launch_bwd_16_dropout(const DropBwdParams& p, hipStream_t stream, const char** name);
hipError_t launch_dropout_keep_mask(uint8_t* keep, uint32_t B, uint32_t H, uint32_t Sq, uint32_t Skv, const int64_t* rng, uint32_t thresh,
                                    hipStream_t stream);

struct RopeParams {
    const void* src;
    void* dst;
    const float* cos_table;
    const float* sin_table;
    int64_t src_batch_stride, src_head_stride, src_seq_stride;
    int64_t table_batch_stride;
    uint32_t B, H, S, D;
    int negate_sin;
};
hipError_t launch_rope(const RopeParams& p, int prec, hipStream_t stream);
hipError_t launch_hadamard(void* data, uint32_t block_size, uint32_t num_blocks, int prec, hipStream_t stream);

struct DequantParams {
    const void* src;
    float* dst;
    void* dst16;
    uint32_t* overflow;
    const float* block_scales;
    const int32_t* block_zero_points;
    uint32_t B, H_src, H_dst, S, D, block_size;
    float scale;
    int zero_point;
    int prec;
    int transposed;
    uint32_t* amax_word;
    const uint32_t* unit_amax;
};
hipError_t launch_dequant(const DequantParams& p, hipStream_t stream);
constexpr uint32_t VSC_HDR_WORDS = 128, VSC_HDR_DEPART = 64, VSC_HDR_SCALE = 65, VSC_HDR_AMAX = 66;
hipError_t launch_cast_rows_bf16_to_f16(const void* src, const int64_t* strides, void* dst, uint32_t B, uint32_t H, uint32_t S, uint32_t D,
                                        uint32_t* hdr, hipStream_t stream);
hipError_t launch_bwd16_rowc(const float* lse, const float* dvec, float* rowc, int64_t n, const float* d_mul , hipStream_t stream);
hipError_t launch_cast_f16_unit(const void* src, int prec, void* dst, int64_t n, uint32_t* hdr, hipStream_t stream, bool amax_done = false );
hipError_t launch_amax_dense(const void* src, int prec, int64_t n, uint32_t* word, hipStream_t stream);
hipError_t launch_amax_dense_n(int count , const void* const* src, int prec, const int64_t* n, uint32_t* const* word, hipStream_t stream);
hipError_t launch_bwd_units(uint32_t* hdr, hipStream_t stream, uint32_t* clean_flag = nullptr);
hipError_t launch_group_sum(const float* src, void* dst, uint32_t B, uint32_t H, uint32_t Hkv, int64_t slab, hipStream_t stream,
                            int out_prec = P_FP32);

struct QuantViews {
    const int8_t* q8;
    const int8_t* k8;
    const void* v16;
    const uint8_t* v8;
    const uint32_t* v_e8;
    const float* q_scale;
    const float* k_scale;
    const float* v_scale;
    const float* qf;
    const float* kf;
    const float* vf;
    const void* qh;
    const void* kh;
    const void* vh;
    uint32_t nqblk, nkblk, dpq;
};
bool quantized_supported(uint32_t D);
size_t quant_workspace_bytes(uint32_t B, uint32_t H, uint32_t Sq, uint32_t Skv, uint32_t D, bool want_f32);
// ... 34 lines not shown
```

universal-metal-flash-attention_amd/csrc/runtime.hip:

```cpp
#include <string>

#include "runtime_internal.h"

using namespace umfa;
using namespace umfa_rt;

namespace umfa_rt {
const bool g_debug = [] {
    const char* e = getenv("MFA_DEBUG");
    return e && e[0] == '1';
}();
std::mutex g_ctx_mu;
Context* g_ctx = nullptr;

bool normalise_mask(const int64_t* shape, const int64_t* strides, uint32_t ndim, int type, int scalar,
                    FwdParams& p) {
    p.mask_kind = MK_NONE;
    for (int i = 0; i < 4; ++i) p.ms[i] = 0;
    if (type == MFA_MASK_TYPE_NONE || ndim == 0 || ndim > 4 || !shape || !strides) return false;
    for (uint32_t i = 0; i < ndim; ++i) {
        const int coord = 4 - (int)ndim + (int)i;
        p.ms[coord] = shape[i] == 1 ? 0 : strides[i];
    }
    if (type == MFA_MASK_TYPE_BOOL) p.mask_kind = MK_BOOL;
    else if (type == MFA_MASK_TYPE_ADDITIVE) {
        p.mask_kind = scalar == MFA_MASK_SCALAR_FP32 ? MK_F32
                      : scalar == MFA_MASK_SCALAR_FP16 ? MK_F16
                      : scalar == MFA_MASK_SCALAR_BF16 ? MK_BF16
                                                       : MK_NONE;
    }
    return p.mask_kind != MK_NONE;
}
}

namespace {

int parse_precision(const char* s) {
    if (!s) return MFA_PRECISION_FP32;
    std::string t(s);
    for (auto& ch : t) ch = (char)tolower(ch);
    if (t == "fp16" || t == "float16") return MFA_PRECISION_FP16;
    if (t == "bf16" || t == "bfloat16") return MFA_PRECISION_BF16;
    if (t == "fp32" || t == "float32") return MFA_PRECISION_FP32;
    if (t == "int8") return MFA_PRECISION_INT8;
    if (t == "int4") return MFA_PRECISION_INT4;
    return MFA_PRECISION_FP32;
}


void dense_strides(FwdParams& p, bool tq, bool tk, bool tv, bool to) {
    auto set = [](int64_t* s, uint32_t H, uint32_t S, uint32_t D, bool t) {
        s[0] = (int64_t)H * S * D;
        s[1] = (int64_t)S * D;
        s[2] = t ? 1 : D;
        s[3] = t ? S : 1;
    };
    set(p.qs, p.H, p.Sq, p.D, tq);
    set(p.ks, p.H, p.Skv, p.D, tk);
    set(p.vs, p.H, p.Skv, p.D, tv);
    p.os[0] = to ? 1 : p.D;
    p.os[1] = to ? p.Sq : 1;
}

mfa_error_t rc_of(hipError_t e) {
    return e == hipSuccess ? MFA_SUCCESS
           : e == hipErrorInvalidValue ? MFA_ERROR_INVALID_ARGS
           : e == hipErrorOutOfMemory ? MFA_ERROR_MEMORY_ALLOCATION
                                      : MFA_ERROR_EXECUTION_FAILED;
}

const char* both_kernels(const char* first, const char* second) {
    static std::map<std::pair<const char*, const char*>, std::string> names;
    std::string& s = names[std::make_pair(first, second)];
    if (s.empty()) s = std::string(first) + " | " + second + " (fp32 mask: chosen on the device)";
    return s.c_str();
}

hipError_t dispatch_forward(Context* ctx, StreamScratch& sc, const FwdParams& p, int intermediate_prec, hipStream_t stream) {
    const char* name = "none";
    hipError_t e = hipSuccess;
    const bool lowp = p.in_prec != P_FP32 && intermediate_prec != P_FP32;
    FwdParams pv = p;
    if (lowp && p.in_prec == P_BF16 && tuning().pv_fp16.load(std::memory_order_relaxed)) pv.pv16 = 1;
    auto cast_v = [&](FwdParams& q, void* mask_scratch = nullptr, CastRowsCall* defer = nullptr) -> bool {
        const uint32_t vB = p.vs[0] == 0 ? 1u : p.B, vH = p.vs[1] == 0 ? 1u : p.H;
        const size_t slabs = (size_t)vB * vH, vbytes = slabs * p.Skv * p.D * 2;
        char* blk = sc.ensure_v16(slabs, vbytes, stream);
        if (!blk) return false;
        void* v16 = blk + sc.v16_cnt_bytes;
        if (defer) {
            *defer = CastRowsCall{p.v, {p.vs[0], p.vs[1], p.vs[2], p.vs[3]}, v16, vB, vH, p.Skv, p.D, (uint32_t*)blk};
            e = hipSuccess;
        } else {
            e = mask_scratch ? launch_cast_rows_and_mask_pack(p.v, p.vs, v16, vB, vH, p.Skv, p.D, (uint32_t*)blk, q, mask_scratch, stream)
                             : launch_cast_rows_bf16_to_f16(p.v, p.vs, v16, vB, vH, p.Skv, p.D, (uint32_t*)blk, stream);
        }
        if (e != hipSuccess) return false;
        q.v = v16;
        q.vs[0] = p.vs[0] == 0 ? 0 : (int64_t)vH * p.Skv * p.D; q.vs[1] = p.vs[1] == 0 ? 0 : (int64_t)p.Skv * p.D; q.vs[2] = p.D; q.vs[3] = 1;
        q.vsc = (const float*)blk;
        q.vsc_bs = p.vs[0] == 0 ? 0u : vH; q.vsc_hs = p.vs[1] == 0 ? 0u : 1u;
        q.pv16 = 2;
        return true;
    };
    bool done = false;
    const uint32_t* guard = nullptr;
    const char* guarded_first = nullptr;
    FwdParams v16_from;
    bool have_v16 = false;
    if (lowp && fwd_w64_supported(pv)) {
        FwdParams pw = pv;
        const bool mask_f32 = pw.mask_kind == MK_F32;
        const bool mask_add = pw.mask_kind == MK_F16 || pw.mask_kind == MK_BF16 || mask_f32;
        const bool mask_w64 = pw.mask_kind == MK_BOOL || mask_add;
        void* mk = mask_w64 ? sc.mflags.ensure(((mask_pack_bytes(pw) + 255) & ~(size_t)255) + mask_copy_bytes(pw), stream) : nullptr;
        bool ok = !mask_w64 || mk != nullptr;
        const FwdW64Plan plan = fwd_w64_plan(pw);
        char* w64 = ok ? sc.ensure_w64(plan.cnt_bytes, plan.buf_bytes, stream) : nullptr;
        ok = ok && w64 != nullptr;
        bool packed = false;
        CastRowsCall cast_call;
        const bool cast_rides = mask_add && mk != nullptr;
        bool cast_deferred = false;
        if (ok && pv.pv16) {
            ok = cast_v(pw, pw.mask_kind == MK_BOOL ? mk : nullptr, cast_rides ? &cast_call : nullptr);
            if (!ok && e != hipSuccess) return e;
            packed = ok && mk != nullptr && pw.mask_kind == MK_BOOL;
            cast_deferred = ok && cast_rides;
        }
        if (ok) {
            if (mk && !packed && (e = (mask_add ? launch_mask_classify(pw, mk, stream, cast_deferred ? &cast_call : nullptr) : launch_mask_pack(pw, mk, stream))) != hipSuccess) return e;
            e = launch_fwd_w64(pw, (float*)(w64 + sc.w64_cnt_bytes), (uint32_t*)w64, stream, &name);
            if (mask_f32) {
                if (e != hipSuccess) return e;
                guard = pw.guard;
                guarded_first = name;
                if (pw.pv16 == 2) { v16_from = pw; have_v16 = true; }
            } else {
                done = true;
            }
        } else if (p.rope_cos || !fwd_16_supported(p)) {
            return hipErrorOutOfMemory;
        }
    }
    if (done) {
    } else if (p.rope_cos) {
        return hipErrorNotSupported;
    } else if (lowp && fwd_16_supported(p)) {
        FwdParams pp = pv;
        if (guard) { pp.guard = guard; pp.guard_want = 1; }
        if (have_v16) {
            pp.v = v16_from.v; pp.vsc = v16_from.vsc; pp.vsc_bs = v16_from.vsc_bs; pp.vsc_hs = v16_from.vsc_hs; pp.pv16 = 2;
            for (int i = 0; i < 4; ++i) pp.vs[i] = v16_from.vs[i];
        } else if (pp.pv16 && (size_t)(p.vs[0] == 0 ? 1u : p.B) * (p.vs[1] == 0 ? 1u : p.H) * p.Skv * p.D * 2 >= ((size_t)16 << 20) && p.Sq >= 1024) {
            if (!cast_v(pp) && e != hipSuccess) return e;
        }
        const FwdSplitPlan plan = fwd_16_split_plan(p);
        pp.decode_form = plan.decode;
        if (plan.nsplit > 1) {
            char* buf = sc.ensure_split(plan.cnt_bytes, plan.buf_bytes, stream);
            if (!buf) return hipErrorOutOfMemory;
            pp.n_full = plan.n_full;
            pp.nsplit = plan.nsplit;
            pp.part_cnt = (uint32_t*)buf;
            pp.part_buf = (float*)(buf + sc.split_cnt_bytes);
        } else if (plan.cbal) {
            if (char* buf = sc.ensure_split(plan.cnt_bytes, plan.buf_bytes, stream)) {
                pp.cbal = 1;
                pp.cbal_delta = plan.cbal_delta;
                pp.part_cnt = (uint32_t*)buf;
                pp.part_buf = (float*)(buf + sc.split_cnt_bytes);
            }
        }
        void* realign_blk = nullptr;
        if (!guard && mask_rows_scalar(pp) && !tuning().no_mask_realign.load(std::memory_order_relaxed)) {
            const size_t fb = (mask_flags_bytes(pp) + 255) & ~(size_t)255, rbytes = mask_realign_bytes(pp);
            if (rbytes <= ((size_t)1 << 30)) {
                if (void* blk = sc.mflags.ensure(fb + rbytes, stream)) {
                    if ((e = launch_mask_realign(pp, (char*)blk + fb, stream)) != hipSuccess) return e;
                    realign_blk = blk;
                }
            }
        }
        if (guard) {
            uint8_t* const fl = (uint8_t*)const_cast<uint32_t*>(guard) + 256;
            const size_t fb = (mask_flags_bytes(pp) + 255) & ~(size_t)255;
            if (mask_rows_scalar(pp) && !tuning().no_mask_realign.load(std::memory_order_relaxed) && mask_realign_bytes(pp) <= ((size_t)1 << 30)) {
                if ((e = launch_mask_realign(pp, fl + fb, stream)) != hipSuccess) return e;
            }
            if (!tuning().no_mask_flags.load(std::memory_order_relaxed)) mask_flags_describe(pp, fl);
        } else if (pp.mask_kind != MK_NONE && !tuning().no_mask_flags.load(std::memory_order_relaxed) && mask_flags_worthwhile(pp)) {
            void* fl = realign_blk ? realign_blk : sc.mflags.ensure(mask_flags_bytes(pp), stream);
            if (fl && launch_mask_flags(pp, (uint8_t*)fl, stream) != hipSuccess) pp.mask_flags = nullptr;
        }
        e = launch_fwd_16(pp, stream, &name);
        if (guard && e == hipSuccess) name = both_kernels(guarded_first, name);
    } else {
        e = p.D > 256 ? launch_fwd_wide(p, stream, &name) : launch_fwd_exact(p, stream, &name);
    }
    ctx->last_kernel = name;
    DBG("forward B%u H%u Sq%u Skv%u D%u causal%d mask%d -> %s (%s)", p.B, p.H, p.Sq, p.Skv, p.D, p.causal,
        p.mask_kind, name, hipGetErrorString(e));
    return e;
}

mfa_error_t forward_sync_chunked(Context* ctx, Buffer* bq, Buffer* bk, Buffer* bv, Buffer* bo, Buffer* bl, const FwdParams& p, int inter, uint32_t want) {
    const std::vector<SyncChunk> chunks = plan_sync_chunks(p.B, p.H, want);
    if (!sync_chunks_begin(ctx, chunks.size())) return MFA_ERROR_EXECUTION_FAILED;
// ... 341 lines not shown
                                     void* mask_buffer, int64_t mask_offset, const int64_t* mask_shape,
                                     const int64_t* mask_strides, uint32_t mask_ndim, mfa_mask_type_t mask_type,
                                     mfa_mask_scalar_t mask_scalar_type, uint32_t batch_size, uint32_t seq_len_q,
                                     uint32_t seq_len_kv, uint32_t num_heads, uint16_t head_dim, float softmax_scale,
                                     bool causal, const char* input_precision, const char* intermediate_precision) {
    if (!as_ctx(context) || !q_buffer || !k_buffer || !v_buffer || !out_buffer) return MFA_ERROR_INVALID_ARGS;
    if (q_offset < 0 || k_offset < 0 || v_offset < 0 || out_offset < 0) return MFA_ERROR_INVALID_ARGS;
    const void* mask = nullptr;
    if (mask_type != MFA_MASK_TYPE_NONE) {
        if (!mask_buffer || mask_offset < 0) return MFA_ERROR_INVALID_ARGS;
        mask = (const char*)mask_buffer + mask_offset;
    }
    return umfa_attention_forward_stream(
        context, command_buffer, (const char*)q_buffer + q_offset, q_strides, (const char*)k_buffer + k_offset,
        k_strides, (const char*)v_buffer + v_offset, v_strides, (char*)out_buffer + out_offset, MFA_PRECISION_FP32,
        nullptr, mask, mask_shape, mask_strides, mask_ndim, mask_type, mask_scalar_type, batch_size, seq_len_q,
        seq_len_kv, num_heads, head_dim, softmax_scale, causal, parse_precision(input_precision),
        parse_precision(intermediate_precision));
}

const char* mfa_error_string(mfa_error_t error) {
    const char* s = "Unknown error";
    switch (error) {
    case 0: s = "Success"; break;
    case 1: s = "Invalid arguments"; break;
    case 2: s = "Memory allocation failed"; break;
    case 3: s = "Device not supported"; break;
    case 4: s = "Kernel compilation failed"; break;
    case 5: s = "Execution failed"; break;
    }
    return strdup(s);
}

bool mfa_is_device_supported(void) { return device_usable(nullptr); }

void mfa_get_version(int* major, int* minor, int* patch) {
    if (major) *major = 1;
    if (minor) *minor = 0;
    if (patch) *patch = 0;
}

double mfa_get_gpu_latency(mfa_context_t context) {
    Context* c = as_ctx(context);
    return c ? c->last_latency : 0.0;
}

int32_t mfa_has_native_bfloat(void) { return device_usable(nullptr) ? 1 : 0; }
int32_t mfa_has_native_bfloat_msl32(void) { return device_usable(nullptr) ? 1 : 0; }

const char* umfa_last_kernel_name(mfa_context_t context) {
    Context* c = as_ctx(context);
    return c ? c->last_kernel : "none";
}

mfa_error_t umfa_release_scratch(mfa_context_t context, void* stream, int32_t all_streams) {
    Context* c = as_ctx(context);
    if (!c) return MFA_ERROR_INVALID_ARGS;
    std::lock_guard<std::mutex> lock(c->mu);
    int n = 0, prev = 0;
    if (hipGetDeviceCount(&n) == hipSuccess && hipGetDevice(&prev) == hipSuccess) {
        for (auto& kv : c->pools)
            if (all_streams || kv.first.stream == (hipStream_t)stream) {
                (void)hipSetDevice(kv.first.dev);
                (void)hipDeviceSynchronize();
            }
        (void)hipSetDevice(prev);
    }
    c->release_pools((hipStream_t)stream, all_streams != 0);
    if (all_streams) mirror_cache().clear();
    return MFA_SUCCESS;
}

mfa_error_t umfa_set_option(mfa_context_t context, const char* name, const char* value) {
    Context* c = as_ctx(context);
    if (!c) return MFA_ERROR_INVALID_ARGS;
    if (!set_tuning(name, value)) return MFA_ERROR_INVALID_ARGS;
    return MFA_SUCCESS;
}

mfa_error_t umfa_get_option(mfa_context_t context, const char* name, char* value, size_t value_size) {
    Context* c = as_ctx(context);
    if (!c || !name || !value || value_size < 2) return MFA_ERROR_INVALID_ARGS;
    if (!strcmp(name, "pv_fp16_status") || !strcmp(name, "pv_fp16_fallbacks")) { value[0] = '0'; value[1] = 0; return MFA_SUCCESS; }
    return get_tuning(name, value, value_size) ? MFA_SUCCESS : MFA_ERROR_INVALID_ARGS;
}

mfa_error_t mfa_set_scale_arrays(mfa_context_t context, const float* q_scales, uint32_t q_scales_count,
                                 const float* k_scales, uint32_t k_scales_count, const float* v_scales,
                                 uint32_t v_scales_count) {
    Context* c = as_ctx(context);
    if (!c) return MFA_ERROR_INVALID_ARGS;
    std::lock_guard<std::mutex> lock(c->mu);
    auto set = [](std::vector<float>& dst, const float* src, uint32_t n) {
        if (src && n) dst.assign(src, src + n);
        else dst.clear();
    };
    set(c->q_scales, q_scales, q_scales_count);
    set(c->k_scales, k_scales, k_scales_count);
    set(c->v_scales, v_scales, v_scales_count);
    return MFA_SUCCESS;
}

void mfa_get_quantized_layout(mfa_quantized_kernel_t, mfa_quantized_layout_t* out_layout) {
    if (!out_layout) return;
    int32_t* f = (int32_t*)out_layout;
    for (size_t i = 0; i < sizeof(mfa_quantized_layout_t) / sizeof(int32_t); ++i) f[i] = -1;
}

void mfa_get_quantized_capabilities(void* out_capabilities) {
    if (!out_capabilities) return;
    mfa_quantized_capabilities_t caps;
    memset(&caps, 0, sizeof(caps));
    caps.supports_multi_head_backward = true;
    caps.supports_blockwise_backward = true;
    caps.max_heads = 128;
    caps.max_block_size = 256;
    memcpy(out_capabilities, &caps, sizeof(caps));
}

mfa_error_t mfa_attention_forward_quantized_direct(
    mfa_context_t context, mfa_buffer_t q, mfa_buffer_t k, mfa_buffer_t v, mfa_buffer_t out, uint32_t batch_size,
    uint32_t seq_len_q, uint32_t seq_len_kv, uint32_t num_heads, uint16_t head_dim, float softmax_scale, bool causal,
    float, int32_t, float, int32_t, float, int32_t, int32_t, int32_t, int32_t, int32_t, bool transpose_q,
    bool transpose_k, bool transpose_v, bool transpose_o) {
    if (!as_ctx(context) || !as_buf(q) || !as_buf(k) || !as_buf(v) || !as_buf(out)) return MFA_ERROR_INVALID_ARGS;
    if (!batch_size || !num_heads || !seq_len_q || !seq_len_kv || !head_dim)
        return MFA_ERROR_MEMORY_ALLOCATION;
    return forward_sync(context, q, k, v, out, nullptr, batch_size, seq_len_q, seq_len_kv, num_heads, head_dim,
                        softmax_scale, causal, MFA_PRECISION_FP32, MFA_PRECISION_FP32, transpose_q, transpose_k,
                        transpose_v, transpose_o, nullptr, 0, nullptr, nullptr, 0, MFA_MASK_TYPE_NONE, 0, false);
}

mfa_error_t mfa_attention_forward_quantized(
    mfa_context_t context, mfa_buffer_t q, mfa_buffer_t k, mfa_buffer_t v, mfa_buffer_t out, uint32_t batch_size,
    uint32_t seq_len_q, uint32_t seq_len_kv, uint32_t num_heads, uint16_t head_dim, float softmax_scale, bool causal,
    float q_scale, int32_t q_zp, float k_scale, int32_t k_zp, float v_scale, int32_t v_zp, mfa_precision_t qp,
    mfa_precision_t kp, mfa_precision_t vp, mfa_precision_t op, bool tq, bool tk, bool tv, bool to) {
    return mfa_attention_forward_quantized_direct(context, q, k, v, out, batch_size, seq_len_q, seq_len_kv, num_heads,
                                                  head_dim, softmax_scale, causal, q_scale, q_zp, k_scale, k_zp,
                                                  v_scale, v_zp, qp, kp, vp, op, tq, tk, tv, to);
}

mfa_error_t mfa_attention_forward_quantized_unified(
    mfa_context_t context, mfa_buffer_t q, mfa_buffer_t k, mfa_buffer_t v, mfa_buffer_t out, uint32_t batch_size,
    uint32_t seq_len_q, uint32_t seq_len_kv, uint32_t num_heads, uint16_t head_dim, float softmax_scale, bool causal,
    float q_scale, int32_t q_zp, float k_scale, int32_t k_zp, float v_scale, int32_t v_zp, mfa_precision_t qp,
    mfa_precision_t kp, mfa_precision_t vp, mfa_precision_t op, int32_t, uint32_t, uint32_t, uint32_t, bool, bool,
    bool tq, bool tk, bool tv, bool to) {
    return mfa_attention_forward_quantized_direct(context, q, k, v, out, batch_size, seq_len_q, seq_len_kv, num_heads,
                                                  head_dim, softmax_scale, causal, q_scale, q_zp, k_scale, k_zp,
                                                  v_scale, v_zp, qp, kp, vp, op, tq, tk, tv, to);
}

mfa_error_t mfa_attention_forward_quantized_enhanced(
    mfa_context_t context, mfa_buffer_t q, mfa_buffer_t k, mfa_buffer_t v, mfa_buffer_t out, uint32_t batch_size,
    uint32_t seq_len_q, uint32_t seq_len_kv, uint32_t num_heads, uint16_t head_dim, float softmax_scale, bool causal,
    float q_scale, int32_t q_zp, float k_scale, int32_t k_zp, float v_scale, int32_t v_zp, mfa_precision_t qp,
    mfa_precision_t kp, mfa_precision_t vp, mfa_precision_t op, int32_t, uint32_t, uint32_t, uint32_t, bool, bool,
    bool tq, bool tk, bool tv, bool to) {
    return mfa_attention_forward_quantized_direct(context, q, k, v, out, batch_size, seq_len_q, seq_len_kv, num_heads,
                                                  head_dim, softmax_scale, causal, q_scale, q_zp, k_scale, k_zp,
                                                  v_scale, v_zp, qp, kp, vp, op, tq, tk, tv, to);
}

mfa_error_t mfa_multihead_attention_quantized_direct(
    mfa_context_t context, mfa_buffer_t q, mfa_buffer_t k, mfa_buffer_t v, mfa_buffer_t out, uint32_t batch_size,
// ... 62 lines not shown
```

universal-metal-flash-attention_amd/csrc/tuning.hip:

```cpp
#include <cstdio>
#include <cstdlib>
#include <cstring>
#include <mutex>
#include <vector>

#include "kernels.h"

namespace umfa {

namespace {
int env_int(const char* name, int dflt) {
    const char* e = getenv(name);
    return (e && *e) ? atoi(e) : dflt;
}
bool env_flag(const char* name) {
    const char* e = getenv(name);
    return e && e[0] == '1';
}
}

Tuning& tuning() {
    static Tuning* t = [] {
        Tuning* x = new Tuning();
        const char* tau = getenv("UMFA_W64_TAU");
        const char* lazy = getenv("UMFA_W64_LAZY");
        if (tau && *tau) {
            const float v = (float)atof(tau);
            if (v >= 0.0f && v <= 16.0f) {
                x->sm_tau.store(v);
                x->sm_mode.store(v == 0.0f ? SM_EXACT : SM_DEFERRED);
            }
        }
        if (lazy && *lazy) x->sm_mode.store(lazy[0] != '0' ? SM_LAZY : (x->sm_mode.load() == SM_DEFAULT ? SM_DEFERRED : x->sm_mode.load()));
        x->force_w64.store(env_flag("UMFA_FORCE_W64"));
        x->no_w64.store(env_flag("UMFA_NO_W64"));
        x->w64_grid.store(env_int("UMFA_W64_GRID", 0));
        x->w64_skew.store(env_int("UMFA_W64_SKEW", 0));
        x->no_mask_flags.store(getenv("UMFA_NO_MASK_FLAGS") != nullptr);
        x->bwd_exact.store(getenv("UMFA_BWD_EXACT") != nullptr);
        x->bwd_dq.store(env_int("UMFA_BWD_DQ", 0));
        x->bwd_persist.store(getenv("UMFA_BWD_PERSIST") != nullptr);
        x->bwd_separate_delta.store(getenv("UMFA_LAB_SEPARATE_DELTA") != nullptr);
        x->no_split.store(env_flag("UMFA_NO_SPLIT"));
        x->force_split.store(env_int("UMFA_FORCE_SPLIT", 0));
        x->no_dma.store(env_flag("UMFA_NO_DMA"));
        x->bn64.store(env_flag("UMFA_BN64"));
        x->pv_fp16.store(env_int("UMFA_PV_FP16", 1) != 0);
        x->bwd_ds_store.store(env_flag("UMFA_BWD_DS_STORE"));
        x->no_w64_mask.store(env_flag("UMFA_NO_W64_MASK"));
        x->ksplit.store(env_flag("UMFA_KSPLIT"));
        x->no_pipe.store(env_flag("UMFA_NO_PIPE"));
        x->no_w64_mask_lazy.store(env_flag("UMFA_NO_W64_MASK_LAZY"));
        x->no_w64_bias.store(env_flag("UMFA_NO_W64_BIAS"));
        x->no_w64_f32_mask.store(env_flag("UMFA_NO_W64_F32_MASK"));
        x->cast_two_pass.store(env_flag("UMFA_CAST_TWO_PASS"));
        x->cast_u.store(env_int("UMFA_CAST_U", 0));
        x->quant_block_wg.store(env_flag("UMFA_QUANT_BLOCK_WG"));
        x->cast_wait_us.store(env_int("UMFA_CAST_WAIT_US", 100));
        x->bwd_ds_lab.store(env_int("UMFA_LAB_DS", 0));
        x->cbal.store(env_int("UMFA_CBAL", 0));
        x->decode_ks.store(env_int("UMFA_DECODE_KS", 0));
        x->cbal_delta.store(env_int("UMFA_CBAL_DELTA", -1));
        x->sync_chunks.store(env_int("UMFA_SYNC_CHUNKS", 1));
        x->sdpa_dropout.store(env_flag("UMFA_SDPA_DROPOUT"));
        return x;
    }();
    return *t;
}

bool set_tuning(const char* name, const char* value) {
    if (!name || !value) return false;
    Tuning& t = tuning();
    const int iv = atoi(value);
    const bool on = value[0] != '\0' && value[0] != '0';
    if (!strcmp(name, "softmax_reference")) {
        const int m = !strcmp(value, "default") ? SM_DEFAULT : !strcmp(value, "exact") ? SM_EXACT
                      : !strcmp(value, "deferred") ? SM_DEFERRED : !strcmp(value, "lazy") ? SM_LAZY : -1;
        if (m < 0) return false;
        t.sm_mode.store(m);
        return true;
    }
    if (!strcmp(name, "softmax_tau") || !strcmp(name, "w64_tau")) {
        const float v = (float)atof(value);
        if (!(v >= 0.0f && v <= 16.0f)) return false;
        t.sm_tau.store(v);
        if (!strcmp(name, "w64_tau")) t.sm_mode.store(v == 0.0f ? SM_EXACT : SM_DEFERRED);
        return true;
    }
    struct { const char* n; std::atomic<int>* v; bool flag; } tab[] = {
        {"force_w64", &t.force_w64, true}, {"no_w64", &t.no_w64, true}, {"w64_grid", &t.w64_grid, false}, {"w64_skew", &t.w64_skew, false},
        {"no_mask_flags", &t.no_mask_flags, true}, {"bwd_exact", &t.bwd_exact, true}, {"bwd_dq", &t.bwd_dq, false},
        {"bwd_persist", &t.bwd_persist, true}, {"bwd_separate_delta", &t.bwd_separate_delta, true},
        {"no_split", &t.no_split, true}, {"force_split", &t.force_split, false}, {"no_dma", &t.no_dma, true},
        {"bn64", &t.bn64, true}, {"pv_fp16", &t.pv_fp16, true}, {"bwd_ds_store", &t.bwd_ds_store, true}, {"no_w64_mask", &t.no_w64_mask, true}, {"ksplit", &t.ksplit, true}, {"no_pipe", &t.no_pipe, true}, {"no_w64_mask_lazy", &t.no_w64_mask_lazy, true}, {"no_w64_bias", &t.no_w64_bias, true}, {"no_w64_f32_mask", &t.no_w64_f32_mask, true}, {"f32_mask_ratio", &t.f32_mask_ratio, false}, {"mask_pass_ratio", &t.mask_pass_ratio, false}, {"no_w64_ragged_mask", &t.no_w64_ragged_mask, true}, {"no_mask_realign", &t.no_mask_realign, true}, {"no_bwd_mask", &t.no_bwd_mask, true}, {"sdpa_dropout", &t.sdpa_dropout, true},
        {"cast_two_pass", &t.cast_two_pass, true}, {"bwd_ds_lab", &t.bwd_ds_lab, false}, {"cast_u", &t.cast_u, false}, {"quant_block_wg", &t.quant_block_wg, true},
        {"cast_wait_us", &t.cast_wait_us, false}, {"cbal", &t.cbal, false}, {"cbal_delta", &t.cbal_delta, false}, {"decode_ks", &t.decode_ks, false}, {"sync_chunks", &t.sync_chunks, false}, {"sync_chunked_calls", &t.sync_chunked_calls, false}, {"mirror_cache_hits", &t.mirror_cache_hits, false},
    };
    for (auto& e : tab)
        if (!strcmp(name, e.n)) {
            e.v->store(e.flag ? (on ? 1 : 0) : iv);
            return true;
        }
    return false;
}

bool get_tuning(const char* name, char* out, size_t n) {
    if (!name || !out || n < 2) return false;
    Tuning& t = tuning();
    char buf[32];
    if (!strcmp(name, "softmax_reference")) {
        const int m = t.sm_mode.load();
        snprintf(buf, sizeof(buf), "%s", m == SM_EXACT ? "exact" : m == SM_DEFERRED ? "deferred" : m == SM_LAZY ? "lazy" : "default");
    } else if (!strcmp(name, "softmax_tau") || !strcmp(name, "w64_tau")) {
        snprintf(buf, sizeof(buf), "%g", (double)t.sm_tau.load());
    } else {
        struct { const char* n; std::atomic<int>* v; } tab[] = {
            {"force_w64", &t.force_w64}, {"no_w64", &t.no_w64}, {"w64_grid", &t.w64_grid}, {"w64_skew", &t.w64_skew},
            {"no_mask_flags", &t.no_mask_flags}, {"bwd_exact", &t.bwd_exact}, {"bwd_dq", &t.bwd_dq}, {"bwd_persist", &t.bwd_persist},
            {"bwd_separate_delta", &t.bwd_separate_delta}, {"no_split", &t.no_split}, {"force_split", &t.force_split},
            {"no_dma", &t.no_dma}, {"bn64", &t.bn64}, {"pv_fp16", &t.pv_fp16}, {"bwd_ds_store", &t.bwd_ds_store}, {"no_w64_mask", &t.no_w64_mask}, {"ksplit", &t.ksplit}, {"no_pipe", &t.no_pipe}, {"no_w64_mask_lazy", &t.no_w64_mask_lazy}, {"no_w64_bias", &t.no_w64_bias}, {"no_w64_f32_mask", &t.no_w64_f32_mask}, {"f32_mask_ratio", &t.f32_mask_ratio}, {"mask_pass_ratio", &t.mask_pass_ratio}, {"no_w64_ragged_mask", &t.no_w64_ragged_mask}, {"no_mask_realign", &t.no_mask_realign}, {"no_bwd_mask", &t.no_bwd_mask}, {"sdpa_dropout", &t.sdpa_dropout},
            {"cast_two_pass", &t.cast_two_pass}, {"bwd_ds_lab", &t.bwd_ds_lab}, {"cast_u", &t.cast_u}, {"quant_block_wg", &t.quant_block_wg},
            {"cast_wait_us", &t.cast_wait_us}, {"cbal", &t.cbal}, {"cbal_delta", &t.cbal_delta}, {"decode_ks", &t.decode_ks}, {"sync_chunks", &t.sync_chunks}, {"sync_chunked_calls", &t.sync_chunked_calls}, {"mirror_cache_hits", &t.mirror_cache_hits},
        };
        const std::atomic<int>* v = nullptr;
        for (auto& e : tab)
            if (!strcmp(name, e.n)) v = e.v;
        if (!v) return false;
        snprintf(buf, sizeof(buf), "%d", v->load());
    }
    if (strlen(buf) + 1 > n) return false;
    strcpy(out, buf);
    return true;
}

int device_cu_count() {
    static std::atomic<int> cus[64];
    int dev = 0;
    if (hipGetDevice(&dev) != hipSuccess || dev < 0 || dev >= 64) dev = 0;
    int n = cus[dev].load(std::memory_order_relaxed);
    if (n <= 0) {
        if (hipDeviceGetAttribute(&n, hipDeviceAttributeMultiprocessorCount, dev) != hipSuccess || n <= 0) n = 256;
        cus[dev].store(n, std::memory_order_relaxed);
    }
    return n;
}

hipError_t ensure_dynamic_lds(const void* kernel, size_t bytes) {
    if (bytes <= 48 * 1024) return hipSuccess;
    struct Entry { const void* k; int dev; size_t bytes; };
    static std::mutex mu;
    static std::vector<Entry> done;
    int dev = 0;
    if (hipGetDevice(&dev) != hipSuccess) dev = 0;
    std::lock_guard<std::mutex> lock(mu);
    for (const Entry& e : done)
        if (e.k == kernel && e.dev == dev && e.bytes >= bytes) return hipSuccess;
    hipError_t e = hipFuncSetAttribute(kernel, hipFuncAttributeMaxDynamicSharedMemorySize, (int)bytes);
    if (e != hipSuccess) return e;
    done.push_back({kernel, dev, bytes});
    return hipSuccess;
}

}
```

universal-metal-flash-attention_amd/umfa_torch/ops.py:

```python
from __future__ import annotations

import ctypes
from typing import Optional, Tuple

import torch

from umfa._ffi import (MFA_MASK_SCALAR_BF16, MFA_MASK_SCALAR_BYTE, MFA_MASK_SCALAR_FP16, MFA_MASK_SCALAR_FP32,
                       MFA_MASK_TYPE_ADDITIVE, MFA_MASK_TYPE_BOOL, MFA_MASK_TYPE_NONE, MFA_PRECISION_BF16,
                       MFA_PRECISION_FP16, MFA_PRECISION_FP32, MFAError, _check_error, _lib, mfa_context_t)

_PREC = {torch.float16: MFA_PRECISION_FP16, torch.bfloat16: MFA_PRECISION_BF16, torch.float32: MFA_PRECISION_FP32}
_PREC_NAME = {torch.float16: b"fp16", torch.bfloat16: b"bf16", torch.float32: b"fp32"}

_ctx = None


def context():
    global _ctx
    if _ctx is None:
        if not torch.cuda.is_available():
            raise RuntimeError("umfa_torch needs a ROCm device: there is no CPU fallback")
        h = mfa_context_t()
        _check_error(_lib.mfa_create_context(ctypes.byref(h)))
        _ctx = h
    return _ctx


def last_kernel() -> str:
    return _lib.umfa_last_kernel_name(context()).decode()


def release_scratch(stream=None, all_streams: bool = False) -> None:
    st = torch.cuda.current_stream().cuda_stream if stream is None else stream.cuda_stream
    _check_error(_lib.umfa_release_scratch(context(), ctypes.c_void_p(st), 1 if all_streams else 0))


_OPTION_NAMES = ("softmax_reference", "softmax_tau", "w64_tau", "force_w64", "no_w64", "w64_grid", "w64_skew", "no_mask_flags", "bwd_exact",
                 "bwd_dq", "bwd_persist", "bwd_separate_delta", "no_split", "force_split", "no_dma", "bn64", "pv_fp16", "bwd_ds_store", "no_w64_mask", "ksplit", "no_pipe", "no_w64_mask_lazy", "no_w64_bias", "no_w64_f32_mask", "f32_mask_ratio", "mask_pass_ratio", "no_w64_ragged_mask", "no_mask_realign",
                 "cast_two_pass", "bwd_ds_lab", "cast_u", "quant_block_wg", "cast_wait_us", "cbal", "cbal_delta", "decode_ks", "sync_chunks", "sync_chunked_calls", "mirror_cache_hits", "no_bwd_mask", "sdpa_dropout")


def get_option(name: str) -> str:
    buf = ctypes.create_string_buffer(64)
    _check_error(_lib.umfa_get_option(context(), name.encode(), buf, 64))
    return buf.value.decode()


def pv_fp16_status() -> int:
    return int(get_option("pv_fp16_status"))


def set_option(name: str, value) -> None:
    _check_error(_lib.umfa_set_option(context(), name.encode(), str(value).encode()))


class options:

    def __init__(self, **kw):
        unknown = [k for k in kw if k not in _OPTION_NAMES]
        if unknown:
            raise KeyError(f"unknown launcher switch(es) {unknown}; known: {_OPTION_NAMES}")
        self.kw = kw
        self.prev = {}

    def __enter__(self):
        prev = {k: get_option(k) for k in self.kw}
        if "w64_tau" in self.kw or "softmax_tau" in self.kw:
            prev.setdefault("softmax_reference", get_option("softmax_reference"))
        for k, v in self.kw.items():
            set_option(k, v)
        self.prev = prev
        return self

    def __exit__(self, *exc):
        ref = self.prev.pop("softmax_reference", None)
        for k, v in self.prev.items():
            set_option("softmax_tau" if k == "w64_tau" else k, v)
        if ref is not None:
            set_option("softmax_reference", ref)
        return False


def _i64(vals):
    return (ctypes.c_int64 * len(vals))(*[int(v) for v in vals])


def _mask_args(mask: Optional[torch.Tensor]):
    if mask is None:
        return None, None, None, 0, MFA_MASK_TYPE_NONE, MFA_MASK_SCALAR_BYTE
    if mask.dtype == torch.bool:
        mt, ms = MFA_MASK_TYPE_BOOL, MFA_MASK_SCALAR_BYTE
    elif mask.dtype == torch.float32:
        mt, ms = MFA_MASK_TYPE_ADDITIVE, MFA_MASK_SCALAR_FP32
    elif mask.dtype == torch.float16:
        mt, ms = MFA_MASK_TYPE_ADDITIVE, MFA_MASK_SCALAR_FP16
    elif mask.dtype == torch.bfloat16:
        mt, ms = MFA_MASK_TYPE_ADDITIVE, MFA_MASK_SCALAR_BF16
    else:
        raise TypeError(f"unsupported mask dtype {mask.dtype}")
    if mask.dim() > 4:
        raise ValueError("attention masks of more than 4 dims are not supported")
    return (ctypes.c_void_p(mask.data_ptr()), _i64(mask.shape), _i64(mask.stride()), mask.dim(), mt, ms)


def _quant_mode(name: str) -> int:
    n = name.lower()
    return 3 if "fp8" in n else 2 if n.startswith("block") else 0


def attention_forward(q: torch.Tensor, k: torch.Tensor, v: torch.Tensor, *, scale: Optional[float] = None,
                      causal: bool = False, mask: Optional[torch.Tensor] = None, out_dtype=None,
                      return_lse: bool = False, intermediate_dtype=None, out: Optional[torch.Tensor] = None,
                      window=None):
    assert q.is_cuda and k.is_cuda and v.is_cuda, "device tensors required"
    B, H, Sq, D = q.shape
    Skv = k.shape[2]
    if scale is None:
        scale = D ** -0.5
    out_dtype = out_dtype or q.dtype
    for t in (q, k, v):
        if t.stride(-1) != 1:
            raise ValueError("last dimension must be contiguous")
# ... 585 lines not shown
```

Measured before the change: 1089.

## Fuse V bf16-to-fp16 cast into the w64 forward attention launch

Moves the per-slab V amax scan and bf16-to-fp16 scaled cast from a separate cast_rows kernel into the w64 forward launch itself. Attention blocks cast V slabs in-line, using write-through stores and a ready flag in the scale header. This removes a kernel launch and the gap between cast and attention for unmasked bf16 D=128 inputs. In exchange it adds cross-block synchronisation inside the attention kernel and some redundant or serialised cast work at the start of the launch. The new path is on by default and can be turned off with an env option.

```diff
diff --git a/universal-metal-flash-attention_amd/csrc/fa_aux.hip b/universal-metal-flash-attention_amd/csrc/fa_aux.hip
--- a/universal-metal-flash-attention_amd/csrc/fa_aux.hip
+++ b/universal-metal-flash-attention_amd/csrc/fa_aux.hip
@@ -1,3 +1,4 @@
+#include "fa_cast_rows.h"
 #include "fa_common.h"
 #include "kernels.h"
 
@@ -486,134 +487,6 @@
     mask_pack_body<VEC16>(p, blockIdx.x);
 }
 
-constexpr uint32_t VH_WORDS = 128, VH_DEPART = 64, VH_SCALE = 65, VH_AMAX = 66;
-__device__ __forceinline__ int vscale_exponent(unsigned amax_bits) {
-    if (amax_bits == 0) return 0;
-    int E = (int)(amax_bits >> 7);
-    E = E > 254 ? 254 : E;
-    const int e = (E ? E - 127 : -126) - 15;
-    return e < -100 ? -100 : e;
-}
-__device__ __forceinline__ unsigned bf16x8_amax(const unsigned (&r)[4], unsigned amax) {
-#pragma unroll
-    for (int j = 0; j < 4; ++j) {
-        const unsigned a = r[j] & 0x7fff7fffu, m2 = (a & 0xffffu) > (a >> 16) ? (a & 0xffffu) : (a >> 16);
-        amax = amax > m2 ? amax : m2;
-    }
-    return amax;
-}
-__device__ __forceinline__ unsigned wave_umax(unsigned x) {
-#pragma unroll
-    for (int off = 32; off > 0; off >>= 1) {
-        const unsigned o2 = (unsigned)__shfl_xor((int)x, off, 64);
-        x = x > o2 ? x : o2;
-    }
-    return x;
-}
-__device__ __forceinline__ unsigned block_amax(unsigned amax, unsigned* wmax) {
-    amax = wave_umax(amax);
-    if ((threadIdx.x & 63) == 0) wmax[threadIdx.x >> 6] = amax;
-    __syncthreads();
-    unsigned m = wmax[0];
-    for (int w = 1; w < 4; ++w) m = m > wmax[w] ? m : wmax[w];
-    return m;
-}
-
-struct CastRowsArgs {
-    const uint16_t* src;
-    int64_t sb, sh, ss;
-    _Float16* dst;
-    uint32_t H, S, D8, chunks;
-    uint32_t* hdr;
-    uint32_t wait_ticks;
-};
-template <int U, bool FUSED>
-__device__ __forceinline__ void cast_rows_body(const CastRowsArgs& a, const uint32_t block) {
-    const uint16_t* __restrict__ src = a.src;
-    _Float16* __restrict__ dst = a.dst;
-    uint32_t* __restrict__ hdr = a.hdr;
-    const int64_t sb = a.sb, sh = a.sh, ss = a.ss;
-    const uint32_t H = a.H, S = a.S, D8 = a.D8, chunks = a.chunks;
-    typedef unsigned u32x4 __attribute__((ext_vector_type(4)));
-    __shared__ unsigned wmax[4], slab_amax;
-    const uint32_t bh = block / chunks, chunk = block - bh * chunks, b = bh / H, h = bh - b * H;
-    const uint32_t rpw = 256u / D8;
-    const uint32_t tr = threadIdx.x / D8, c = threadIdx.x - tr * D8;
-    const uint32_t row0 = chunk * (U * rpw) + tr;
-    const uint16_t* sp = src + (int64_t)b * sb + (int64_t)h * sh + 8 * c;
-    _Float16* dp = dst + ((int64_t)bh * S) * (8 * D8) + 8 * c;
-    uint32_t* const hw = hdr + VH_WORDS * (size_t)bh;
-    u32x4 raw[U];
-#pragma unroll
-    for (int u = 0; u < U; ++u) {
-        const uint32_t r = row0 + u * rpw;
-        raw[u] = r < S && tr < rpw ? __builtin_nontemporal_load((const u32x4*)(sp + (int64_t)r * ss)) : u32x4{0, 0, 0, 0};
-    }
-    unsigned amax;
-    if constexpr (FUSED) {
-        amax = 0;
-#pragma unroll
-        for (int u = 0; u < U; ++u) {
-            const unsigned r4[4] = {raw[u][0], raw[u][1], raw[u][2], raw[u][3]};
-            amax = bf16x8_amax(r4, amax);
-        }
-        amax = block_amax(amax, wmax);
-        if (threadIdx.x < 64) {
-            if (threadIdx.x == 0) __hip_atomic_store(hw + chunk, 0x80000000u | amax, __ATOMIC_RELAXED, __HIP_MEMORY_SCOPE_AGENT);
-            const uint64_t t_in = __builtin_amdgcn_s_memrealtime();
-            unsigned f;
-            bool served = true;
-            for (;;) {
-                f = threadIdx.x < chunks ? __hip_atomic_load(hw + threadIdx.x, __ATOMIC_RELAXED, __HIP_MEMORY_SCOPE_AGENT) : 0x80000000u;
-                if (__builtin_amdgcn_ballot_w64((f & 0x80000000u) == 0) == 0) break;
-                if (__builtin_amdgcn_s_memrealtime() - t_in >= a.wait_ticks) { served = false; break; }
-                __builtin_amdgcn_s_sleep(2);
-            }
-            f = wave_umax(f & 0x7fffffffu);
-            if (threadIdx.x == 0) slab_amax = served ? f : 0xffffffffu;
-        }
-        __syncthreads();
-        if (slab_amax == 0xffffffffu) {
-            for (uint32_t r = tr; r < S && tr < rpw; r += rpw) {
-                const u32x4 v = *(const u32x4*)(sp + (int64_t)r * ss);
-                const unsigned r4[4] = {v[0], v[1], v[2], v[3]};
-                amax = bf16x8_amax(r4, amax);
-            }
-            __syncthreads();
-            amax = block_amax(amax, wmax);
-        } else {
-            amax = slab_amax;
-        }
-    } else {
-        amax = hw[VH_AMAX];
-    }
-    const int e = vscale_exponent(amax);
-    const float mul = __uint_as_float((unsigned)(127 - e) << 23);
-#pragma unroll
-    for (int u = 0; u < U; ++u) {
-        const uint32_t r = row0 + u * rpw;
-        u32x4 o;
-#pragma unroll
-        for (int j = 0; j < 4; ++j) {
-            const float lo = __uint_as_float(raw[u][j] << 16) * mul, hi = __uint_as_float(raw[u][j] & 0xffff0000u) * mul;
-            asm("v_cvt_pk_f16_f32 %0, %1, %2" : "=v"(o[j]) : "v"(lo), "v"(hi));
-        }
-        if (r < S && tr < rpw) *(u32x4*)(dp + (int64_t)r * (8 * D8)) = o;
-    }
-    if (threadIdx.x < 64) {
-        unsigned d = 0;
-        if (threadIdx.x == 0) d = __hip_atomic_fetch_add(hw + VH_DEPART, 1u, __ATOMIC_RELAXED, __HIP_MEMORY_SCOPE_AGENT);
-        d = (unsigned)__builtin_amdgcn_readfirstlane((int)d);
-        if (d == chunks - 1) {
-            if (FUSED && threadIdx.x < chunks) __hip_atomic_store(hw + threadIdx.x, 0u, __ATOMIC_RELAXED, __HIP_MEMORY_SCOPE_AGENT);
-            if (threadIdx.x == 0) {
-                hw[VH_SCALE] = (unsigned)(127 + e) << 23;
-                __hip_atomic_store(hw + VH_DEPART, 0u, __ATOMIC_RELAXED, __HIP_MEMORY_SCOPE_AGENT);
-                if (!FUSED) __hip_atomic_store(hw + VH_AMAX, 0u, __ATOMIC_RELAXED, __HIP_MEMORY_SCOPE_AGENT);
-            }
-        }
-    }
-}
 
 template <int U, bool FUSED>
 __global__ __launch_bounds__(256) void cast_rows_bf16_f16_kernel(CastRowsArgs a) {
diff --git a/universal-metal-flash-attention_amd/csrc/fa_cast_rows.h b/universal-metal-flash-attention_amd/csrc/fa_cast_rows.h
--- /dev/null
+++ b/universal-metal-flash-attention_amd/csrc/fa_cast_rows.h
@@ -0,0 +1,194 @@
+#pragma once
+#include <cstdint>
+
+#include "fa_common.h"
+
+namespace umfa {
+
+constexpr uint32_t VH_WORDS = 128, VH_DEPART = 64, VH_SCALE = 65, VH_AMAX = 66, VH_READY = 67, VH_OUT0 = 96, VH_OUT_TOP = 112, VH_OUT_SHARDS = 16;
+__device__ __forceinline__ int vscale_exponent(unsigned amax_bits) {
+    if (amax_bits == 0) return 0;
+    int E = (int)(amax_bits >> 7);
+    E = E > 254 ? 254 : E;
+    const int e = (E ? E - 127 : -126) - 15;
+    return e < -100 ? -100 : e;
+}
+__device__ __forceinline__ unsigned bf16x8_amax(const unsigned (&r)[4], unsigned amax) {
+#pragma unroll
+    for (int j = 0; j < 4; ++j) {
+        const unsigned a = r[j] & 0x7fff7fffu, m2 = (a & 0xffffu) > (a >> 16) ? (a & 0xffffu) : (a >> 16);
+        amax = amax > m2 ? amax : m2;
+    }
+    return amax;
+}
+__device__ __forceinline__ unsigned wave_umax(unsigned x) {
+#pragma unroll
+    for (int off = 32; off > 0; off >>= 1) {
+        const unsigned o2 = (unsigned)__shfl_xor((int)x, off, 64);
+        x = x > o2 ? x : o2;
+    }
+    return x;
+}
+__device__ __forceinline__ unsigned block_amax(unsigned amax, unsigned* wmax) {
+    amax = wave_umax(amax);
+    if ((threadIdx.x & 63) == 0) wmax[threadIdx.x >> 6] = amax;
+    __syncthreads();
+    unsigned m = wmax[0];
+    for (int w = 1; w < 4; ++w) m = m > wmax[w] ? m : wmax[w];
+    return m;
+}
+
+struct CastRowsArgs {
+    const uint16_t* src;
+    int64_t sb, sh, ss;
+    _Float16* dst;
+    uint32_t H, S, D8, chunks;
+    uint32_t* hdr;
+    uint32_t wait_ticks;
+};
+__device__ __forceinline__ void store16_through(void* dst, const unsigned __attribute__((ext_vector_type(4))) v) {
+    asm volatile("global_store_dwordx4 %0, %1, off sc1" ::"v"(dst), "v"(v) : "memory");
+}
+template <int U, bool FUSED, bool INL = false>
+__device__ __forceinline__ void cast_rows_body(const CastRowsArgs& a, const uint32_t block, unsigned* ex = nullptr) {
+    const uint16_t* __restrict__ src = a.src;
+    _Float16* __restrict__ dst = a.dst;
+    uint32_t* __restrict__ hdr = a.hdr;
+    const int64_t sb = a.sb, sh = a.sh, ss = a.ss;
+    const uint32_t H = a.H, S = a.S, D8 = a.D8, chunks = a.chunks;
+    typedef unsigned u32x4 __attribute__((ext_vector_type(4)));
+    unsigned* wmax;
+    unsigned* slab_amax_p;
+    if constexpr (INL) {
+        wmax = ex;
+        slab_amax_p = ex + 4;
+    } else {
+        __shared__ unsigned wmax_s[4], slab_amax_s;
+        wmax = wmax_s;
+        slab_amax_p = &slab_amax_s;
+    }
+    unsigned& slab_amax = *slab_amax_p;
+    const uint32_t bh = block / chunks, chunk = block - bh * chunks, b = bh / H, h = bh - b * H;
+    const uint32_t rpw = 256u / D8;
+    const uint32_t tr = threadIdx.x / D8, c = threadIdx.x - tr * D8;
+    const uint32_t row0 = chunk * (U * rpw) + tr;
+    const uint16_t* sp = src + (int64_t)b * sb + (int64_t)h * sh + 8 * c;
+    _Float16* dp = dst + ((int64_t)bh * S) * (8 * D8) + 8 * c;
+    uint32_t* const hw = hdr + VH_WORDS * (size_t)bh;
+    u32x4 raw[U];
+#pragma unroll
+    for (int u = 0; u < U; ++u) {
+        const uint32_t r = row0 + u * rpw;
+        raw[u] = r < S && tr < rpw ? __builtin_nontemporal_load((const u32x4*)(sp + (int64_t)r * ss)) : u32x4{0, 0, 0, 0};
+    }
+    unsigned amax;
+    if constexpr (FUSED) {
+        amax = 0;
+#pragma unroll
+        for (int u = 0; u < U; ++u) {
+            const unsigned r4[4] = {raw[u][0], raw[u][1], raw[u][2], raw[u][3]};
+            amax = bf16x8_amax(r4, amax);
+        }
+        amax = block_amax(amax, wmax);
+        if (threadIdx.x < 64) {
+            if (threadIdx.x == 0) __hip_atomic_store(hw + chunk, 0x80000000u | amax, __ATOMIC_RELAXED, __HIP_MEMORY_SCOPE_AGENT);
+            const uint64_t t_in = __builtin_amdgcn_s_memrealtime();
+            unsigned f;
+            bool served = true;
+            for (;;) {
+                f = threadIdx.x < chunks ? __hip_atomic_load(hw + threadIdx.x, __ATOMIC_RELAXED, __HIP_MEMORY_SCOPE_AGENT) : 0x80000000u;
+                if (__builtin_amdgcn_ballot_w64((f & 0x80000000u) == 0) == 0) break;
+                if (__builtin_amdgcn_s_memrealtime() - t_in >= a.wait_ticks) { served = false; break; }
+                __builtin_amdgcn_s_sleep(2);
+            }
+            f = wave_umax(f & 0x7fffffffu);
+            if (threadIdx.x == 0) slab_amax = served ? f : 0xffffffffu;
+        }
+        __syncthreads();
+        if (slab_amax == 0xffffffffu) {
+            for (uint32_t r = tr; r < S && tr < rpw; r += rpw) {
+                const u32x4 v = *(const u32x4*)(sp + (int64_t)r * ss);
+                const unsigned r4[4] = {v[0], v[1], v[2], v[3]};
+                amax = bf16x8_amax(r4, amax);
+            }
+            __syncthreads();
+            amax = block_amax(amax, wmax);
+        } else {
+            amax = slab_amax;
+        }
+    } else {
+        amax = hw[VH_AMAX];
+    }
+    const int e = vscale_exponent(amax);
+    const float mul = __uint_as_float((unsigned)(127 - e) << 23);
+#pragma unroll
+    for (int u = 0; u < U; ++u) {
+        const uint32_t r = row0 + u * rpw;
+        u32x4 o;
+#pragma unroll
+        for (int j = 0; j < 4; ++j) {
+            const float lo = __uint_as_float(raw[u][j] << 16) * mul, hi = __uint_as_float(raw[u][j] & 0xffff0000u) * mul;
+            asm("v_cvt_pk_f16_f32 %0, %1, %2" : "=v"(o[j]) : "v"(lo), "v"(hi));
+        }
+        if (r < S && tr < rpw) {
+            if constexpr (INL) store16_through(dp + (int64_t)r * (8 * D8), o);
+            else *(u32x4*)(dp + (int64_t)r * (8 * D8)) = o;
+        }
+    }
+    if constexpr (INL) {
+        asm volatile("s_waitcnt vmcnt(0)" ::: "memory");
+        __syncthreads();
+    }
+    if (threadIdx.x < 64) {
+        unsigned d = 0;
+        if (threadIdx.x == 0) d = __hip_atomic_fetch_add(hw + VH_DEPART, 1u, __ATOMIC_RELAXED, __HIP_MEMORY_SCOPE_AGENT);
+        d = (unsigned)__builtin_amdgcn_readfirstlane((int)d);
+        if (d == chunks - 1) {
+            if (FUSED && threadIdx.x < chunks) __hip_atomic_store(hw + threadIdx.x, 0u, __ATOMIC_RELAXED, __HIP_MEMORY_SCOPE_AGENT);
+            if (threadIdx.x == 0) {
+                if constexpr (INL) __hip_atomic_store(hw + VH_SCALE, (unsigned)(127 + e) << 23, __ATOMIC_RELAXED, __HIP_MEMORY_SCOPE_AGENT);
+                else hw[VH_SCALE] = (unsigned)(127 + e) << 23;
+                __hip_atomic_store(hw + VH_DEPART, 0u, __ATOMIC_RELAXED, __HIP_MEMORY_SCOPE_AGENT);
+                if (!FUSED) __hip_atomic_store(hw + VH_AMAX, 0u, __ATOMIC_RELAXED, __HIP_MEMORY_SCOPE_AGENT);
+            }
+            if constexpr (INL) {
+                asm volatile("s_waitcnt vmcnt(0)" ::: "memory");
+                if (threadIdx.x == 0) __hip_atomic_store(hw + VH_READY, 1u, __ATOMIC_RELAXED, __HIP_MEMORY_SCOPE_AGENT);
+            }
+        }
+    }
+}
+
+__device__ __forceinline__ void cast_slab_self(const CastRowsArgs& a, const uint32_t bh, unsigned* wmax_self) {
+    typedef unsigned u32x4 __attribute__((ext_vector_type(4)));
+    const uint32_t H = a.H, S = a.S, D8 = a.D8, b = bh / H, h = bh - b * H;
+    const uint32_t rpw = 256u / D8, tr = threadIdx.x / D8, c = threadIdx.x - tr * D8;
+    const uint16_t* sp = a.src + (int64_t)b * a.sb + (int64_t)h * a.sh + 8 * c;
+    _Float16* dp = a.dst + ((int64_t)bh * S) * (8 * D8) + 8 * c;
+    unsigned amax = 0;
+#pragma unroll 1
+    for (uint32_t r = tr; r < S && tr < rpw; r += rpw) {
+        const u32x4 v = *(const u32x4*)(sp + (int64_t)r * a.ss);
+        const unsigned r4[4] = {v[0], v[1], v[2], v[3]};
+        amax = bf16x8_amax(r4, amax);
+    }
+    amax = block_amax(amax, wmax_self);
+    const int e = vscale_exponent(amax);
+    const float mul = __uint_as_float((unsigned)(127 - e) << 23);
+#pragma unroll 1
+    for (uint32_t r = tr; r < S && tr < rpw; r += rpw) {
+        const u32x4 v = *(const u32x4*)(sp + (int64_t)r * a.ss);
+        u32x4 o;
+#pragma unroll
+        for (int j = 0; j < 4; ++j) {
+            const float lo = __uint_as_float(v[j] << 16) * mul, hi = __uint_as_float(v[j] & 0xffff0000u) * mul;
+            asm("v_cvt_pk_f16_f32 %0, %1, %2" : "=v"(o[j]) : "v"(lo), "v"(hi));
+        }
+        store16_through(dp + (int64_t)r * (8 * D8), o);
+    }
+    if (threadIdx.x == 0) __hip_atomic_store(a.hdr + VH_WORDS * (size_t)bh + VH_SCALE, (unsigned)(127 + e) << 23, __ATOMIC_RELAXED, __HIP_MEMORY_SCOPE_AGENT);
+    asm volatile("s_waitcnt vmcnt(0)" ::: "memory");
+    __syncthreads();
+}
+
+}
diff --git a/universal-metal-flash-attention_amd/csrc/fa_common.h b/universal-metal-flash-attention_amd/csrc/fa_common.h
--- a/universal-metal-flash-attention_amd/csrc/fa_common.h
+++ b/universal-metal-flash-attention_amd/csrc/fa_common.h
@@ -61,6 +61,9 @@
     const uint32_t* guard;
     uint32_t guard_want;
     uint32_t mask_padded;
+    const void* cast_src;
+    int64_t cast_ss[3];
+    uint32_t cast_B, cast_H;
 };
 
 __device__ __forceinline__ void rope_rotate8(const float (&x)[8], const f32x4& c0, const f32x4& c1, const f32x4& s0,
diff --git a/universal-metal-flash-attention_amd/csrc/fa_fwd16_w64.hip b/universal-metal-flash-attention_amd/csrc/fa_fwd16_w64.hip
--- a/universal-metal-flash-attention_amd/csrc/fa_fwd16_w64.hip
+++ b/universal-metal-flash-attention_amd/csrc/fa_fwd16_w64.hip
@@ -367,6 +367,14 @@
 
 uint32_t fwd_w64_grid(const FwdParams& p) { return w64_grid(p); }
 
+bool fwd_w64_casts_in_launch(const FwdParams& p) {
+    if (!tuning().cast_in_launch.load(std::memory_order_relaxed) || tuning().cast_two_pass.load(std::memory_order_relaxed)) return false;
+    const int lab_u = tuning().cast_u.load(std::memory_order_relaxed);
+    if (lab_u != 0 && lab_u != 16) return false;
+    if (p.in_prec != P_BF16 || !p.pv16 || p.D != 128 || p.mask_kind != MK_NONE || p.rope_cos) return false;
+    return ((uint64_t)p.Skv + 255) / 256 <= 64;
+}
+
 FwdW64Plan fwd_w64_plan(const FwdParams& p) {
     FwdW64Plan plan;
     const uint32_t items = p.B * p.H * ((p.Sq + 255) / 256);
@@ -402,6 +410,16 @@
     wp.rope_cos = p.rope_cos; wp.rope_sin = p.rope_sin; wp.rope_tb = p.rope_tb;
     wp.vsc = p.vsc; wp.vsc_bs = p.vsc_bs; wp.vsc_hs = p.vsc_hs;
     if (p.in_prec == P_BF16 && p.pv16 && !p.vsc) return hipErrorInvalidValue;
+    wp.cast = CastRowsArgs{};
+    wp.cast_slabs = 0;
+    if (p.cast_src) {
+        if (!fwd_w64_casts_in_launch(p) || p.pv16 != 2) return hipErrorInvalidValue;
+        const uint32_t D8 = p.D / 8, rpw = 256u / D8;
+        wp.cast = CastRowsArgs{(const uint16_t*)p.cast_src, p.cast_ss[0], p.cast_ss[1], p.cast_ss[2], (_Float16*)const_cast<void*>(p.v), p.cast_H, p.Skv, D8,
+                               (p.Skv + 16 * rpw - 1) / (16 * rpw), (uint32_t*)const_cast<float*>(p.vsc),
+                               (uint32_t)std::min<int64_t>(std::max(tuning().cast_wait_us.load(std::memory_order_relaxed), 0), 1000000) * 100u};
+        wp.cast_slabs = p.cast_B * p.cast_H;
+    }
     wp.Tw = wp.T; wp.win_left = wp.win_right = 0;
     const bool rope = p.rope_cos != nullptr, window = w64_is_window(p), fp32o = p.out_prec == P_FP32, maska = p.mask_kind == MK_F16, maskt = p.mask_kind == MK_BOOL || maska;
     wp.mask = nullptr; wp.mask_s[0] = wp.mask_s[1] = wp.mask_s[2] = 0;
diff --git a/universal-metal-flash-attention_amd/csrc/fa_fwd16_w64_kernel.inc b/universal-metal-flash-attention_amd/csrc/fa_fwd16_w64_kernel.inc
--- a/universal-metal-flash-attention_amd/csrc/fa_fwd16_w64_kernel.inc
+++ b/universal-metal-flash-attention_amd/csrc/fa_fwd16_w64_kernel.inc
@@ -61,6 +61,9 @@
 #endif
 #ifndef W64_DP
 #define W64_DP 128
+#endif
+#ifndef W64_VSC
+#define W64_VSC 0
 #endif
 #ifndef W64_MSUM_ON
 #define W64_MSUM_ON 0
@@ -398,6 +401,25 @@
     (void)ROPE_ON;
 #endif
 
+#if !W64_I8 && W64_VSC == 1 && W64_DP == 128
+    constexpr bool CAST_INL = !ROPE && !WINDOW && !MASKT;
+#else
+    constexpr bool CAST_INL = false;
+#endif
+    bool cast_on = false, cast_self = false;
+    constexpr unsigned CAST_EX_OFF = 65536u + 4u * 32u * (512u + 16u) + 32u;
+    (void)CAST_EX_OFF;
+#if !W64_I8
+    if constexpr (CAST_INL) {
+        cast_on = p.cast.src != nullptr;
+        if (cast_on) {
+            const uint32_t cast_jobs = p.cast_slabs * p.cast.chunks;
+            for (uint32_t cj = w; cj < cast_jobs; cj += G) cast_rows_body<16, true, true>(p.cast, cj, (unsigned*)(smem + CAST_EX_OFF));
+        }
+    }
+#endif
+    (void)cast_on; (void)CAST_INL;
+
     for (uint32_t si = 0; si < nseg; ++si) {
         int tid_s = tid;
         if constexpr (MASKA) asm volatile("" : "+v"(tid_s));
@@ -453,6 +475,19 @@
         const uint32_t bh = item / nqb, qblk = item % nqb;
         const uint32_t b = bh / p.H, h = bh % p.H;
         const uint32_t q0 = qblk * 256 + (uint32_t)uw * 64;
+#if !W64_I8
+        const bool cast_mine = cast_self;
+        if constexpr (CAST_INL) {
+            if (cast_self) {
+                cast_self = false;
+                cast_slab_self(p.cast, b * p.vsc_bs + h * p.vsc_hs, (unsigned*)(smem + CAST_EX_OFF));
+                __builtin_amdgcn_fence(__ATOMIC_ACQUIRE, "agent");
+                if (tid == 0) *(volatile uint32_t LDS_AS*)(uintptr_t)(lds0 + 65536u + 4u * 32u * (512u + 16u) + 16u) = 1u;
+                __builtin_amdgcn_s_waitcnt(0xc07f);
+            }
+        }
+        (void)cast_mine;
+#endif
 
 #if W64_I8
         (void)b; (void)h;
@@ -702,7 +737,33 @@
 #endif
         W64_L_ZERO();
 #endif
+#if !W64_I8
+        constexpr unsigned CAST_OK_OFF = 65536u + 4u * 32u * (512u + 16u) + 16u;
+        if constexpr (CAST_INL) {
+            if (cast_on && !cast_mine && uw == 0) {
+                uint32_t* const rw = p.cast.hdr + VH_WORDS * ((size_t)b * p.vsc_bs + (size_t)h * p.vsc_hs) + VH_READY;
+                const uint64_t t_in = __builtin_amdgcn_s_memrealtime();
+                unsigned ok = 1u;
+                while (__builtin_amdgcn_readfirstlane((int)__hip_atomic_load(rw, __ATOMIC_RELAXED, __HIP_MEMORY_SCOPE_AGENT)) == 0) {
+                    if (__builtin_amdgcn_s_memrealtime() - t_in >= p.cast.wait_ticks) { ok = 0u; break; }
+                    __builtin_amdgcn_s_sleep(4);
+                }
+                __builtin_amdgcn_fence(__ATOMIC_ACQUIRE, "agent");
+                if (lane == 0) *(volatile uint32_t LDS_AS*)(uintptr_t)(lds0 + CAST_OK_OFF) = ok;
+                __builtin_amdgcn_s_waitcnt(0xc07f);
+            }
+        }
+#endif
         asm volatile("s_waitcnt vmcnt(0)\n\ts_barrier" ::: "memory");
+#if !W64_I8
+        if constexpr (CAST_INL) {
+            if (cast_on && __builtin_amdgcn_readfirstlane((int)*(volatile uint32_t LDS_AS*)(uintptr_t)(lds0 + CAST_OK_OFF)) == 0) {
+                cast_self = true;
+                --si;
+                continue;
+            }
+        }
+#endif
         __builtin_amdgcn_s_waitcnt(0x0F70);
 #pragma unroll
         for (int ks = 0; ks < 4; ++ks) kf[0][ks] = k_frag(0, ks);
@@ -1288,6 +1349,31 @@
         fold_qb(std::integral_constant<int, 0>{});
         fold_qb(std::integral_constant<int, 1>{});
     }
+#if !W64_I8
+    if constexpr (CAST_INL) {
+        if (cast_on && uw == 0) {
+            uint32_t* const ch = p.cast.hdr;
+            const uint32_t slabs = p.cast_slabs;
+            const uint32_t shw = (G + VH_OUT_SHARDS - 1) / VH_OUT_SHARDS, nsh = (G + shw - 1) / shw, sh_i = w / shw;
+            const uint32_t sh_n = G - sh_i * shw < shw ? G - sh_i * shw : shw;
+            uint32_t* const sw = ch + VH_WORDS * (size_t)(sh_i % slabs) + VH_OUT0 + sh_i / slabs;
+            unsigned d = 0;
+            if (lane == 0) d = __hip_atomic_fetch_add(sw, 1u, __ATOMIC_RELAXED, __HIP_MEMORY_SCOPE_AGENT);
+            d = (unsigned)__builtin_amdgcn_readfirstlane((int)d);
+            if (d == sh_n - 1) {
+                if (lane == 0) {
+                    __hip_atomic_store(sw, 0u, __ATOMIC_RELAXED, __HIP_MEMORY_SCOPE_AGENT);
+                    d = __hip_atomic_fetch_add(ch + VH_OUT_TOP, 1u, __ATOMIC_RELAXED, __HIP_MEMORY_SCOPE_AGENT);
+                }
+                d = (unsigned)__builtin_amdgcn_readfirstlane((int)d);
+                if (d == nsh - 1) {
+                    if (lane == 0) __hip_atomic_store(ch + VH_OUT_TOP, 0u, __ATOMIC_RELAXED, __HIP_MEMORY_SCOPE_AGENT);
+                    for (uint32_t i = (uint32_t)lane; i < slabs; i += 64u) __hip_atomic_store(ch + VH_WORDS * (size_t)i + VH_READY, 0u, __ATOMIC_RELAXED, __HIP_MEMORY_SCOPE_AGENT);
+                }
+            }
+        }
+    }
+#endif
 #ifdef W64_LAB_STAMPS
     asm volatile("s_waitcnt vmcnt(0)" ::: "memory");
     W64_STAMP(st_epi);
diff --git a/universal-metal-flash-attention_amd/csrc/fa_fwd16_w64_params.h b/universal-metal-flash-attention_amd/csrc/fa_fwd16_w64_params.h
--- a/universal-metal-flash-attention_amd/csrc/fa_fwd16_w64_params.h
+++ b/universal-metal-flash-attention_amd/csrc/fa_fwd16_w64_params.h
@@ -1,6 +1,7 @@
 #pragma once
 #include <cstdint>
 
+#include "fa_cast_rows.h"
 #include "fa_common.h"
 #include "fa_fwd_16_kernel.h"
 #include "kernels.h"
@@ -37,6 +38,8 @@
     const float* vsc;
     uint32_t vsc_bs, vsc_hs;
     const uint32_t* guard;
+    CastRowsArgs cast;
+    uint32_t cast_slabs;
 };
 
 #include "fa_fwd16_w64_regs.inc"
diff --git a/universal-metal-flash-attention_amd/csrc/kernels.h b/universal-metal-flash-attention_amd/csrc/kernels.h
--- a/universal-metal-flash-attention_amd/csrc/kernels.h
+++ b/universal-metal-flash-attention_amd/csrc/kernels.h
@@ -26,6 +26,7 @@
         cast_u{0} ,
         quant_block_wg{0} ,
         cast_wait_us{100} ,
+        cast_in_launch{1} ,
         decode_ks{0} ,
         cbal{0} ,
         cbal_delta{-1} ,
@@ -65,6 +66,7 @@
 double fwd_16_predict_us(const FwdParams& p);
 FwdW64Plan fwd_w64_plan(const FwdParams& p);
 hipError_t launch_fwd_w64(const FwdParams& p, float* part_buf, uint32_t* part_cnt, hipStream_t stream, const char** name);
+bool fwd_w64_casts_in_launch(const FwdParams& p);
 
 hipError_t launch_bwd(const BwdParams& p, hipStream_t stream, const char** name);
 bool bwd_16_supported(const BwdParams& p);
diff --git a/universal-metal-flash-attention_amd/csrc/runtime.hip b/universal-metal-flash-attention_amd/csrc/runtime.hip
--- a/universal-metal-flash-attention_amd/csrc/runtime.hip
+++ b/universal-metal-flash-attention_amd/csrc/runtime.hip
@@ -82,13 +82,19 @@
     const bool lowp = p.in_prec != P_FP32 && intermediate_prec != P_FP32;
     FwdParams pv = p;
     if (lowp && p.in_prec == P_BF16 && tuning().pv_fp16.load(std::memory_order_relaxed)) pv.pv16 = 1;
-    auto cast_v = [&](FwdParams& q, void* mask_scratch = nullptr, CastRowsCall* defer = nullptr) -> bool {
+    auto cast_v = [&](FwdParams& q, void* mask_scratch = nullptr, CastRowsCall* defer = nullptr, bool in_launch = false) -> bool {
         const uint32_t vB = p.vs[0] == 0 ? 1u : p.B, vH = p.vs[1] == 0 ? 1u : p.H;
         const size_t slabs = (size_t)vB * vH, vbytes = slabs * p.Skv * p.D * 2;
         char* blk = sc.ensure_v16(slabs, vbytes, stream);
         if (!blk) return false;
         void* v16 = blk + sc.v16_cnt_bytes;
-        if (defer) {
+        if (in_launch) {
+            if (!p.v || p.vs[3] != 1 || (p.vs[0] | p.vs[1] | p.vs[2]) % 8 || ((uintptr_t)p.v & 15)) { e = hipErrorInvalidValue; return false; }
+            q.cast_src = p.v;
+            q.cast_ss[0] = p.vs[0]; q.cast_ss[1] = p.vs[1]; q.cast_ss[2] = p.vs[2];
+            q.cast_B = vB; q.cast_H = vH;
+            e = hipSuccess;
+        } else if (defer) {
             *defer = CastRowsCall{p.v, {p.vs[0], p.vs[1], p.vs[2], p.vs[3]}, v16, vB, vH, p.Skv, p.D, (uint32_t*)blk};
             e = hipSuccess;
         } else {
@@ -123,7 +129,8 @@
         const bool cast_rides = mask_add && mk != nullptr;
         bool cast_deferred = false;
         if (ok && pv.pv16) {
-            ok = cast_v(pw, pw.mask_kind == MK_BOOL ? mk : nullptr, cast_rides ? &cast_call : nullptr);
+            ok = cast_v(pw, pw.mask_kind == MK_BOOL ? mk : nullptr, cast_rides ? &cast_call : nullptr,
+                        !mask_w64 && fwd_w64_casts_in_launch(pw));
             if (!ok && e != hipSuccess) return e;
             packed = ok && mk != nullptr && pw.mask_kind == MK_BOOL;
             cast_deferred = ok && cast_rides;
@@ -631,6 +638,20 @@
     Context* c = as_ctx(context);
     if (!c || !name || !value || value_size < 2) return MFA_ERROR_INVALID_ARGS;
     if (!strcmp(name, "pv_fp16_status") || !strcmp(name, "pv_fp16_fallbacks")) { value[0] = '0'; value[1] = 0; return MFA_SUCCESS; }
+    if (!strcmp(name, "cast_header_words")) {
+        std::lock_guard<std::mutex> lock(c->mu);
+        size_t bad = 0;
+        for (auto& kv : c->pools) {
+            StreamScratch& s = kv.second;
+            if (!s.v16.ptr || !s.v16_cnt_bytes) continue;
+            DeviceGuard g(kv.first.dev);
+            std::vector<uint32_t> h(s.v16_cnt_bytes / 4);
+            if (hipDeviceSynchronize() != hipSuccess || hipMemcpy(h.data(), s.v16.ptr, h.size() * 4, hipMemcpyDeviceToHost) != hipSuccess) return MFA_ERROR_EXECUTION_FAILED;
+            for (size_t i = 0; i < h.size(); ++i) bad += (i % VSC_HDR_WORDS != VSC_HDR_SCALE && h[i] != 0u) ? 1 : 0;
+        }
+        snprintf(value, value_size, "%zu", bad);
+        return MFA_SUCCESS;
+    }
     return get_tuning(name, value, value_size) ? MFA_SUCCESS : MFA_ERROR_INVALID_ARGS;
 }
 
diff --git a/universal-metal-flash-attention_amd/csrc/tuning.hip b/universal-metal-flash-attention_amd/csrc/tuning.hip
--- a/universal-metal-flash-attention_amd/csrc/tuning.hip
+++ b/universal-metal-flash-attention_amd/csrc/tuning.hip
@@ -57,6 +57,7 @@
         x->cast_u.store(env_int("UMFA_CAST_U", 0));
         x->quant_block_wg.store(env_flag("UMFA_QUANT_BLOCK_WG"));
         x->cast_wait_us.store(env_int("UMFA_CAST_WAIT_US", 100));
+        x->cast_in_launch.store(env_int("UMFA_CAST_IN_LAUNCH", 1) != 0);
         x->bwd_ds_lab.store(env_int("UMFA_LAB_DS", 0));
         x->cbal.store(env_int("UMFA_CBAL", 0));
         x->decode_ks.store(env_int("UMFA_DECODE_KS", 0));
@@ -94,7 +95,7 @@
         {"no_split", &t.no_split, true}, {"force_split", &t.force_split, false}, {"no_dma", &t.no_dma, true},
         {"bn64", &t.bn64, true}, {"pv_fp16", &t.pv_fp16, true}, {"bwd_ds_store", &t.bwd_ds_store, true}, {"no_w64_mask", &t.no_w64_mask, true}, {"ksplit", &t.ksplit, true}, {"no_pipe", &t.no_pipe, true}, {"no_w64_mask_lazy", &t.no_w64_mask_lazy, true}, {"no_w64_bias", &t.no_w64_bias, true}, {"no_w64_f32_mask", &t.no_w64_f32_mask, true}, {"f32_mask_ratio", &t.f32_mask_ratio, false}, {"mask_pass_ratio", &t.mask_pass_ratio, false}, {"no_w64_ragged_mask", &t.no_w64_ragged_mask, true}, {"no_mask_realign", &t.no_mask_realign, true}, {"no_bwd_mask", &t.no_bwd_mask, true}, {"sdpa_dropout", &t.sdpa_dropout, true},
         {"cast_two_pass", &t.cast_two_pass, true}, {"bwd_ds_lab", &t.bwd_ds_lab, false}, {"cast_u", &t.cast_u, false}, {"quant_block_wg", &t.quant_block_wg, true},
-        {"cast_wait_us", &t.cast_wait_us, false}, {"cbal", &t.cbal, false}, {"cbal_delta", &t.cbal_delta, false}, {"decode_ks", &t.decode_ks, false}, {"sync_chunks", &t.sync_chunks, false}, {"sync_chunked_calls", &t.sync_chunked_calls, false}, {"mirror_cache_hits", &t.mirror_cache_hits, false},
+        {"cast_in_launch", &t.cast_in_launch, true}, {"cast_wait_us", &t.cast_wait_us, false}, {"cbal", &t.cbal, false}, {"cbal_delta", &t.cbal_delta, false}, {"decode_ks", &t.decode_ks, false}, {"sync_chunks", &t.sync_chunks, false}, {"sync_chunked_calls", &t.sync_chunked_calls, false}, {"mirror_cache_hits", &t.mirror_cache_hits, false},
     };
     for (auto& e : tab)
         if (!strcmp(name, e.n)) {
@@ -120,7 +121,7 @@
             {"bwd_separate_delta", &t.bwd_separate_delta}, {"no_split", &t.no_split}, {"force_split", &t.force_split},
             {"no_dma", &t.no_dma}, {"bn64", &t.bn64}, {"pv_fp16", &t.pv_fp16}, {"bwd_ds_store", &t.bwd_ds_store}, {"no_w64_mask", &t.no_w64_mask}, {"ksplit", &t.ksplit}, {"no_pipe", &t.no_pipe}, {"no_w64_mask_lazy", &t.no_w64_mask_lazy}, {"no_w64_bias", &t.no_w64_bias}, {"no_w64_f32_mask", &t.no_w64_f32_mask}, {"f32_mask_ratio", &t.f32_mask_ratio}, {"mask_pass_ratio", &t.mask_pass_ratio}, {"no_w64_ragged_mask", &t.no_w64_ragged_mask}, {"no_mask_realign", &t.no_mask_realign}, {"no_bwd_mask", &t.no_bwd_mask}, {"sdpa_dropout", &t.sdpa_dropout},
             {"cast_two_pass", &t.cast_two_pass}, {"bwd_ds_lab", &t.bwd_ds_lab}, {"cast_u", &t.cast_u}, {"quant_block_wg", &t.quant_block_wg},
-            {"cast_wait_us", &t.cast_wait_us}, {"cbal", &t.cbal}, {"cbal_delta", &t.cbal_delta}, {"decode_ks", &t.decode_ks}, {"sync_chunks", &t.sync_chunks}, {"sync_chunked_calls", &t.sync_chunked_calls}, {"mirror_cache_hits", &t.mirror_cache_hits},
+            {"cast_in_launch", &t.cast_in_launch}, {"cast_wait_us", &t.cast_wait_us}, {"cbal", &t.cbal}, {"cbal_delta", &t.cbal_delta}, {"decode_ks", &t.decode_ks}, {"sync_chunks", &t.sync_chunks}, {"sync_chunked_calls", &t.sync_chunked_calls}, {"mirror_cache_hits", &t.mirror_cache_hits},
         };
         const std::atomic<int>* v = nullptr;
         for (auto& e : tab)
diff --git a/universal-metal-flash-attention_amd/umfa_torch/ops.py b/universal-metal-flash-attention_amd/umfa_torch/ops.py
--- a/universal-metal-flash-attention_amd/umfa_torch/ops.py
+++ b/universal-metal-flash-attention_amd/umfa_torch/ops.py
@@ -37,7 +37,7 @@
 
 _OPTION_NAMES = ("softmax_reference", "softmax_tau", "w64_tau", "force_w64", "no_w64", "w64_grid", "w64_skew", "no_mask_flags", "bwd_exact",
                  "bwd_dq", "bwd_persist", "bwd_separate_delta", "no_split", "force_split", "no_dma", "bn64", "pv_fp16", "bwd_ds_store", "no_w64_mask", "ksplit", "no_pipe", "no_w64_mask_lazy", "no_w64_bias", "no_w64_f32_mask", "f32_mask_ratio", "mask_pass_ratio", "no_w64_ragged_mask", "no_mask_realign",
-                 "cast_two_pass", "bwd_ds_lab", "cast_u", "quant_block_wg", "cast_wait_us", "cbal", "cbal_delta", "decode_ks", "sync_chunks", "sync_chunked_calls", "mirror_cache_hits", "no_bwd_mask", "sdpa_dropout")
+                 "cast_two_pass", "bwd_ds_lab", "cast_u", "quant_block_wg", "cast_wait_us", "cast_in_launch", "cbal", "cbal_delta", "decode_ks", "sync_chunks", "sync_chunked_calls", "mirror_cache_hits", "no_bwd_mask", "sdpa_dropout")
 
 
 def get_option(name: str) -> str:
```

New measurement: 1046. 0.96x the previous value.
